# tqch/ddpm-torch

Hardware: AMD Instinct MI355X
Metric: training imgs/s/GPU + 1000-step DDPM samples/s, CIFAR-10 UNet @1/2/4/8 MI355X (higher is better)
Workload: dtype bf16; 1 GPU; configs/cifar10.json UNet (35.7M params), full Trainer.step, B=128 per GPU, 32x32, T=1000, dropout 0.1, Adam+clip+EMA; global_batch=128, rccl_ranks=1, parallelism=dp1

## Files before the change

ddpm-torch_amd/csrc/common.h:

```cpp
#pragma once
#include <hip/hip_runtime.h>
#include <hip/hip_ext.h>
#include <stdint.h>

#define DDPM_OK 0
#define DDPM_ERR_SHAPE 1
#define DDPM_ERR_DTYPE 2
#define DDPM_ERR_ALIGN 3
#define DDPM_ERR_LAUNCH 4
#define DDPM_ERR_NULL 5

#define DDPM_F32 0
#define DDPM_BF16 1

typedef unsigned short bf16_t;

typedef float f32x4 __attribute__((ext_vector_type(4)));
typedef float f32x16 __attribute__((ext_vector_type(16)));
typedef short s16x8 __attribute__((ext_vector_type(8)));
typedef unsigned int u32x4 __attribute__((ext_vector_type(4)));

__device__ __forceinline__ float bf2f(bf16_t v) { return __uint_as_float(((unsigned)v) << 16); }
typedef __attribute__((ext_vector_type(2))) __bf16 hw_bf16x2;
typedef __attribute__((ext_vector_type(2))) float hw_f32x2;
__device__ __forceinline__ unsigned pack_bf2(float lo, float hi) {
    hw_f32x2 v; v.x = lo; v.y = hi;
    return __builtin_bit_cast(unsigned, __builtin_convertvector(v, hw_bf16x2));
}
__device__ __forceinline__ bf16_t f2bf(float f) { return (bf16_t)(pack_bf2(f, 0.f) & 0xffffu); }

template <typename T> struct Elem;
template <> struct Elem<float> {
    static constexpr int VEC = 4;
    __device__ static __forceinline__ float ld(const float* p) { return *p; }
    __device__ static __forceinline__ void st(float* p, float v) { *p = v; }
    __device__ static __forceinline__ void unpack(const u32x4& v, float* f) {
        f[0] = __uint_as_float(v.x); f[1] = __uint_as_float(v.y); f[2] = __uint_as_float(v.z); f[3] = __uint_as_float(v.w);
    }
    __device__ static __forceinline__ u32x4 pack(const float* f) {
        u32x4 v; v.x = __float_as_uint(f[0]); v.y = __float_as_uint(f[1]); v.z = __float_as_uint(f[2]); v.w = __float_as_uint(f[3]);
        return v;
    }
};
template <> struct Elem<bf16_t> {
    static constexpr int VEC = 8;
    __device__ static __forceinline__ float ld(const bf16_t* p) { return bf2f(*p); }
    __device__ static __forceinline__ void st(bf16_t* p, float v) { *p = f2bf(v); }
    __device__ static __forceinline__ void unpack(const u32x4& v, float* f) {
        f[0] = __uint_as_float(v.x << 16); f[1] = __uint_as_float(v.x & 0xffff0000u);
        f[2] = __uint_as_float(v.y << 16); f[3] = __uint_as_float(v.y & 0xffff0000u);
        f[4] = __uint_as_float(v.z << 16); f[5] = __uint_as_float(v.z & 0xffff0000u);
        f[6] = __uint_as_float(v.w << 16); f[7] = __uint_as_float(v.w & 0xffff0000u);
    }
    __device__ static __forceinline__ u32x4 pack(const float* f) {
        u32x4 v; v.x = pack_bf2(f[0], f[1]); v.y = pack_bf2(f[2], f[3]); v.z = pack_bf2(f[4], f[5]); v.w = pack_bf2(f[6], f[7]);
        return v;
    }
};

__device__ __forceinline__ u32x4 ldg16(const void* p) { return *reinterpret_cast<const u32x4*>(p); }
__device__ __forceinline__ void stg16(void* p, const u32x4& v) { *reinterpret_cast<u32x4*>(p) = v; }
__device__ __forceinline__ u32x4 zero16() { u32x4 v; v.x = v.y = v.z = v.w = 0u; return v; }

__device__ __forceinline__ float wave_sum(float v) {
#pragma unroll
    for (int o = 32; o > 0; o >>= 1) v += __shfl_xor(v, o, 64);
    return v;
}
__device__ __forceinline__ float wave_max(float v) {
#pragma unroll
    for (int o = 32; o > 0; o >>= 1) v = fmaxf(v, __shfl_xor(v, o, 64));
    return v;
}

__device__ __forceinline__ float sigmoidf_(float z) { return 1.0f / (1.0f + __expf(-z)); }
__device__ __forceinline__ float siluf_(float z) { return z * sigmoidf_(z); }
__device__ __forceinline__ float silu_fast_(float z) { return z * __builtin_amdgcn_rcpf(1.0f + __expf(-z)); }
__device__ __forceinline__ float silu_gradf_(float z) { float s = sigmoidf_(z); return s * (1.0f + z * (1.0f - s)); }

struct FastDiv {
    unsigned mul, shift, d;
};
__device__ __forceinline__ unsigned fdiv(unsigned n, const FastDiv& f) {
    return (unsigned)(((unsigned long long)n * f.mul) >> f.shift);
}
static inline FastDiv make_fastdiv(unsigned d) {
    FastDiv f; f.d = d ? d : 1; f.mul = 1u << 31; f.shift = 31;
    if (d <= 1) return f;
    unsigned l = 0; while ((1ull << l) < d) ++l;
    f.shift = 31 + l;
    if ((1ull << l) == d) return f;
    f.mul = (unsigned)((1ull << f.shift) / d + 1);
    return f;
}

__device__ __forceinline__ unsigned mix32(unsigned x) {
    x ^= x >> 16; x *= 0x7feb352dU; x ^= x >> 15; x *= 0x846ca68bU; x ^= x >> 16;
    return x;
}
__device__ __forceinline__ unsigned dropout_word(unsigned long long seed, unsigned long long pair) {
    const unsigned lo = (unsigned)pair, hi = (unsigned)(pair >> 32);
    return mix32(lo ^ mix32(hi + (unsigned)seed) ^ (unsigned)(seed >> 32) * 0x9E3779B9u);
}
__device__ __forceinline__ bool dropout_keep(unsigned long long seed, unsigned long long idx, unsigned thresh16) {
    const unsigned w = dropout_word(seed, idx >> 1);
    return ((idx & 1) ? (w >> 16) : (w & 0xffffu)) >= thresh16;
}
__device__ __forceinline__ unsigned dropout_h0(unsigned long long seed) {
    return mix32((unsigned)seed) ^ ((unsigned)(seed >> 32) * 0x9E3779B9u);
}
__device__ __forceinline__ unsigned dropout_word32(unsigned h0, unsigned pair) { return mix32(pair ^ h0); }
static inline unsigned dropout_thresh16(float p) {
    const double th = (double)p * 65536.0;
    return th <= 0 ? 0u : (th >= 65536.0 ? 65536u : (unsigned)(th + 0.5));
}
__device__ __forceinline__ float silu_grad_fast_(float z) {
    const float s = __builtin_amdgcn_rcpf(1.0f + __expf(-z));
    return s * (1.0f + z * (1.0f - s));
}

#include <atomic>
struct DevOnce {
    std::atomic<unsigned long long> mask{0};
    static unsigned long long bit() { int d = 0; (void)hipGetDevice(&d); return 1ull << (d & 63); }
    bool operator!() const { return !(mask.load(std::memory_order_acquire) & bit()); }
    DevOnce& operator=(bool) { mask.fetch_or(bit(), std::memory_order_release); return *this; }
};

struct DdpmLaunchEdge {
    hipStream_t stream = nullptr;
    hipEvent_t event = nullptr;
    bool armed = false;
    bool attached = false;
};
extern thread_local DdpmLaunchEdge g_ddpm_launch_edge;

template <class... P> static inline void ddpm_launch_with_event(DdpmLaunchEdge& edge, void (*kernel)(P...), dim3 grid, dim3 block, unsigned lds,
                                                                hipStream_t st, P... formal) {
    void* args[sizeof...(P) + 1] = {(void*)&formal..., nullptr};
    if (hipExtLaunchKernel((const void*)kernel, grid, block, args, lds, st, nullptr, edge.event, 0) == hipSuccess) edge.attached = true;
}
template <class... P, class... A> static inline void ddpm_launch(void (*kernel)(P...), dim3 grid, dim3 block, unsigned lds, hipStream_t st, A&&... args) {
    static_assert(sizeof...(P) == sizeof...(A), "kernel argument count");
    DdpmLaunchEdge& edge = g_ddpm_launch_edge;
    if (edge.armed && edge.stream == st) ddpm_launch_with_event<P...>(edge, kernel, grid, block, lds, st, static_cast<P>(args)...);
    else kernel<<<grid, block, lds, st>>>(args...);
}
#undef hipLaunchKernelGGL
#define hipLaunchKernelGGL(kernel, grid, block, lds, stream, ...) ddpm_launch(kernel, dim3(grid), dim3(block), (unsigned)(lds), stream, __VA_ARGS__)

static inline int check_launch() { return hipGetLastError() == hipSuccess ? DDPM_OK : DDPM_ERR_LAUNCH; }
static inline bool aligned16(const void* p) { return (((uintptr_t)p) & 15) == 0; }

int ddpm_sumsq_finish_launch(const float* partial, int n, float* total_sq, void* stream);
int ddpm_reserved_cus();
static inline int ddpm_cu_budget(int wanted) { const int left = 256 - ddpm_reserved_cus(); return wanted < left ? wanted : (left > 1 ? left : 1); }
int ddpm_pointwise_launch(const void* x, long long x_ld, const void* w, void* y, long long y_ld, const float* bias, const void* residual,
                          long long res_ld, int accumulate, int M, int N, int K, int dry, void* stream);
int ddpm_edgeconv_few_out_launch(const void* x, long long x_ld, const void* w, void* y, const float* bias, int B, int H, int W, int C, int N,
                                 int dry, void* stream);
int ddpm_edgeconv_few_in_launch(const void* x, long long x_ld, const void* w, void* y, long long y_ld, const float* bias, int B, int H, int W,
                                int C, int N, int dry, void* stream);
int ddpm_conv3x3_stream_launch(const void* x, long long x_ld, const void* w, void* y, long long y_ld, const float* bias, const float* rowbias,
                               long long rowbias_ld, const void* residual, long long res_ld, int accumulate, int B, int H, int W, int C, int N,
                               int upsample, int xcd, int dry, void* stream);
```

ddpm-torch_amd/csrc/elementwise.hip:

```cpp
#include "common.h"
#include <stdlib.h>

static inline int grid_for(long long n, int block = 256, int cap = 256 * 16) {
    long long g = (n + block - 1) / block;
    if (g > cap) g = cap;
    if (g < 1) g = 1;
    return (int)g;
}

__global__ void temb_kernel(const long long* __restrict__ t, const float* __restrict__ freqs, float* __restrict__ out, int B, int dim) {
    const int half = dim / 2;
    for (int i = blockIdx.x * blockDim.x + threadIdx.x; i < B * dim; i += gridDim.x * blockDim.x) {
        const int b = i / dim, j = i - b * dim;
        float v = 0.f;
        if (j < 2 * half) {
            const float arg = __fmul_rn((float)t[b], freqs[j < half ? j : j - half]);
            v = j < half ? sinf(arg) : cosf(arg);
        }
        out[i] = v;
    }
}
extern "C" int ddpm_timestep_embedding(const long long* t, const float* freqs, float* out, int B, int dim, void* stream) {
    if (!t || !out || !freqs) return DDPM_ERR_NULL;
    if (B <= 0 || dim < 4) return DDPM_ERR_SHAPE;
    hipLaunchKernelGGL(temb_kernel, dim3(grid_for((long long)B * dim)), dim3(256), 0, (hipStream_t)stream, t, freqs, out, B, dim);
    return check_launch();
}

template <typename T>
__global__ void nchw_to_nhwc_kernel(const float* __restrict__ x, T* __restrict__ y, int B, int C, int HW, int Cp) {
    const long long n = (long long)B * HW * Cp;
    for (long long i = (long long)blockIdx.x * blockDim.x + threadIdx.x; i < n; i += (long long)gridDim.x * blockDim.x) {
        const int c = (int)(i % Cp);
        const long long bp = i / Cp;
        const int p = (int)(bp % HW);
        const long long b = bp / HW;
        Elem<T>::st(y + i, c < C ? x[(b * C + c) * HW + p] : 0.f);
    }
}
extern "C" int ddpm_nchw_to_nhwc(const float* x, void* y, int B, int C, int HW, int Cp, int dtype, void* stream) {
    if (!x || !y) return DDPM_ERR_NULL;
    if (B <= 0 || C <= 0 || HW <= 0 || Cp < C) return DDPM_ERR_SHAPE;
    const int g = grid_for((long long)B * HW * Cp);
    if (dtype == DDPM_BF16) hipLaunchKernelGGL(nchw_to_nhwc_kernel<bf16_t>, dim3(g), dim3(256), 0, (hipStream_t)stream, x, (bf16_t*)y, B, C, HW, Cp);
    else if (dtype == DDPM_F32) hipLaunchKernelGGL(nchw_to_nhwc_kernel<float>, dim3(g), dim3(256), 0, (hipStream_t)stream, x, (float*)y, B, C, HW, Cp);
    else return DDPM_ERR_DTYPE;
    return check_launch();
}

template <typename T>
__global__ void pack_weight_kernel(const float* __restrict__ w, T* __restrict__ wf, T* __restrict__ wd, int N, int C, int R, int S, int Cp, int Np) {
    const int RS = R * S;
    if (wf) {
        const long long n = (long long)N * RS * Cp;
        for (long long i = (long long)blockIdx.x * blockDim.x + threadIdx.x; i < n; i += (long long)gridDim.x * blockDim.x) {
            const int c = (int)(i % Cp); const long long r1 = i / Cp;
            const int tap = (int)(r1 % RS); const int nn = (int)(r1 / RS);
            Elem<T>::st(wf + i, c < C ? w[((long long)nn * C + c) * RS + tap] : 0.f);
        }
    }
    if (wd) {
        const long long n = (long long)C * RS * Np;
        for (long long i = (long long)blockIdx.x * blockDim.x + threadIdx.x; i < n; i += (long long)gridDim.x * blockDim.x) {
            const int nn = (int)(i % Np); const long long r1 = i / Np;
            const int tap = (int)(r1 % RS); const int c = (int)(r1 / RS);
            Elem<T>::st(wd + i, nn < N ? w[((long long)nn * C + c) * RS + (RS - 1 - tap)] : 0.f);
        }
    }
}
extern "C" int ddpm_pack_weight(const float* w, void* wf, void* wd, int N, int C, int R, int S, int Cp, int Np, int dtype, void* stream) {
    if (!w || (!wf && !wd)) return DDPM_ERR_NULL;
    if (Cp < C || Np < N) return DDPM_ERR_SHAPE;
    const long long big = (long long)(Cp > C ? Cp : C) * R * S * (Np > N ? Np : N);
    const int g = grid_for(big);
    if (dtype == DDPM_BF16) hipLaunchKernelGGL(pack_weight_kernel<bf16_t>, dim3(g), dim3(256), 0, (hipStream_t)stream, w, (bf16_t*)wf, (bf16_t*)wd, N, C, R, S, Cp, Np);
    else if (dtype == DDPM_F32) hipLaunchKernelGGL(pack_weight_kernel<float>, dim3(g), dim3(256), 0, (hipStream_t)stream, w, (float*)wf, (float*)wd, N, C, R, S, Cp, Np);
    else return DDPM_ERR_DTYPE;
    return check_launch();
}

constexpr int PK_T = 32;
template <typename T> __device__ __forceinline__ void pk_store2(T* p, float a, float b);
template <> __device__ __forceinline__ void pk_store2<bf16_t>(bf16_t* p, float a, float b) { *reinterpret_cast<unsigned*>(p) = pack_bf2(a, b); }
template <> __device__ __forceinline__ void pk_store2<float>(float* p, float a, float b) { *reinterpret_cast<float2*>(p) = make_float2(a, b); }

template <typename T, int RS>
__device__ __forceinline__ void pack_tensor(const float* __restrict__ w, T* __restrict__ wf, T* __restrict__ wd, int N, int C, int Cp, int Np, bool up_dgrad,
                                            float* tile) {
    constexpr int pitch = PK_T * RS + 1;
    const int tiles_c = (Cp + PK_T - 1) / PK_T, tiles_n = (Np + PK_T - 1) / PK_T;
    const int tid = threadIdx.x;
    const bool vec_ok = ((long long)C * RS) % 4 == 0 && (((unsigned long long)w) & 15) == 0;
    for (int t = blockIdx.x; t < tiles_c * tiles_n; t += gridDim.x) {
        const int n0 = (t / tiles_c) * PK_T, c0 = (t % tiles_c) * PK_T;
        const int cw = min(PK_T, C - c0);
        __syncthreads();
        constexpr int V = PK_T * RS / 4, KV = PK_T * V / 256;
        static_assert(PK_T * V % 256 == 0, "whole vectors per thread");
        if (cw == PK_T && vec_ok) {
            float4 xv[KV];
#pragma unroll
            for (int k = 0; k < KV; ++k) {
                const int i = tid + 256 * k, nl = i / V, v = i - nl * V;
                xv[k] = n0 + nl < N ? *reinterpret_cast<const float4*>(w + ((long long)(n0 + nl) * C + c0) * RS + 4 * v) : make_float4(0.f, 0.f, 0.f, 0.f);
            }
#pragma unroll
            for (int k = 0; k < KV; ++k) {
                const int i = tid + 256 * k, nl = i / V, v = i - nl * V;
                float* t4 = tile + nl * pitch + 4 * v;
                t4[0] = xv[k].x; t4[1] = xv[k].y; t4[2] = xv[k].z; t4[3] = xv[k].w;
            }
        } else {
            for (int i = tid; i < PK_T * PK_T * RS; i += 256) {
                const int nl = i / (PK_T * RS), rem = i - nl * (PK_T * RS);
                const bool ok = n0 + nl < N && rem < cw * RS;
                tile[nl * pitch + rem] = ok ? w[((long long)(n0 + nl) * C + c0) * RS + rem] : 0.f;
            }
        }
        __syncthreads();
        constexpr bool BF = sizeof(T) == 2;
        if (wf) {
            if constexpr (BF) {
                for (int i = tid; i < PK_T * RS * (PK_T / 8); i += 256) {
                    const int cl = (i % (PK_T / 8)) * 8, r1 = i / (PK_T / 8), tap = r1 % RS, nl = r1 / RS;
                    if (n0 + nl < N && c0 + cl < Cp) {
                        const float* t8 = tile + nl * pitch + cl * RS + tap;
                        u32x4 o;
                        o.x = pack_bf2(t8[0], t8[RS]); o.y = pack_bf2(t8[2 * RS], t8[3 * RS]); o.z = pack_bf2(t8[4 * RS], t8[5 * RS]); o.w = pack_bf2(t8[6 * RS], t8[7 * RS]);
                        *reinterpret_cast<u32x4*>(wf + ((long long)(n0 + nl) * RS + tap) * Cp + c0 + cl) = o;
                    }
                }
            } else {
                for (int i = tid; i < PK_T * RS * (PK_T / 2); i += 256) {
                    const int cl = (i % (PK_T / 2)) * 2, r1 = i / (PK_T / 2), tap = r1 % RS, nl = r1 / RS;
                    if (n0 + nl < N && c0 + cl < Cp)
                        pk_store2<T>(wf + ((long long)(n0 + nl) * RS + tap) * Cp + c0 + cl, tile[nl * pitch + cl * RS + tap], tile[nl * pitch + (cl + 1) * RS + tap]);
                }
            }
        }
        if constexpr (RS == 9) {
            if (wd && up_dgrad) {
                for (int i = tid; i < PK_T * 16 * (PK_T / 2); i += 256) {
                    const int nl = (i % (PK_T / 2)) * 2, r1 = i / (PK_T / 2), tap = r1 % 16, cl = r1 / 16;
                    if (c0 + cl >= C || n0 + nl >= Np) continue;
                    const int P = tap >> 2, Q = tap & 3;
                    float acc0 = 0.f, acc1 = 0.f;
#pragma unroll
                    for (int a = 0; a < 2; ++a)
#pragma unroll
                        for (int b2 = 0; b2 < 2; ++b2) {
                            const int r = P - a, s2 = Q - b2;
                            if (r >= 0 && r < 3 && s2 >= 0 && s2 < 3) {
                                acc0 += tile[nl * pitch + cl * 9 + (8 - (r * 3 + s2))];
                                acc1 += tile[(nl + 1) * pitch + cl * 9 + (8 - (r * 3 + s2))];
                            }
                        }
                    pk_store2<T>(wd + ((long long)(c0 + cl) * 16 + tap) * Np + n0 + nl, acc0, acc1);
                }
                continue;
            }
        }
        if (wd) {
            if constexpr (BF) {
                for (int i = tid; i < PK_T * RS * (PK_T / 8); i += 256) {
                    const int nl = (i % (PK_T / 8)) * 8, r1 = i / (PK_T / 8), tap = r1 % RS, cl = r1 / RS;
                    if (c0 + cl < C && n0 + nl < Np) {
                        const float* t8 = tile + nl * pitch + cl * RS + (RS - 1 - tap);
                        u32x4 o;
                        o.x = pack_bf2(t8[0], t8[pitch]); o.y = pack_bf2(t8[2 * pitch], t8[3 * pitch]); o.z = pack_bf2(t8[4 * pitch], t8[5 * pitch]);
                        o.w = pack_bf2(t8[6 * pitch], t8[7 * pitch]);
                        *reinterpret_cast<u32x4*>(wd + ((long long)(c0 + cl) * RS + tap) * Np + n0 + nl) = o;
                    }
                }
            } else {
                for (int i = tid; i < PK_T * RS * (PK_T / 2); i += 256) {
                    const int nl = (i % (PK_T / 2)) * 2, r1 = i / (PK_T / 2), tap = r1 % RS, cl = r1 / RS;
                    if (c0 + cl < C && n0 + nl < Np)
                        pk_store2<T>(wd + ((long long)(c0 + cl) * RS + tap) * Np + n0 + nl, tile[nl * pitch + cl * RS + (RS - 1 - tap)],
                                     tile[(nl + 1) * pitch + cl * RS + (RS - 1 - tap)]);
                }
            }
        }
    }
}
template <typename T>
__global__ __launch_bounds__(256)
void pack_weight_multi_kernel(const long long* __restrict__ descs) {
    const long long* d = descs + 8 * (long long)blockIdx.y;
    const float* w = reinterpret_cast<const float*>(d[0]);
    T* wf = reinterpret_cast<T*>(d[1]);
    T* wd = reinterpret_cast<T*>(d[2]);
    const int N = (int)d[3], C = (int)d[4], R = (int)d[5] & 0xff, Cp = (int)d[6], Np = (int)d[7];
    const bool up_dgrad = ((int)d[5] & 0x100) != 0;
    __shared__ float tile[PK_T * (PK_T * 9 + 1)];
    if (R == 3) pack_tensor<T, 9>(w, wf, wd, N, C, Cp, Np, up_dgrad, tile);
    else if (R == 1) pack_tensor<T, 1>(w, wf, wd, N, C, Cp, Np, false, tile);
    else if (R == 2) pack_tensor<T, 4>(w, wf, wd, N, C, Cp, Np, false, tile);
}
extern "C" int ddpm_pack_weight_multi(const long long* descs, int n_tensors, int dtype, void* stream) {
    if (!descs) return DDPM_ERR_NULL;
    if (n_tensors <= 0) return DDPM_OK;
    constexpr int pk_blocks = 256;
    if (dtype == DDPM_BF16) hipLaunchKernelGGL(pack_weight_multi_kernel<bf16_t>, dim3(pk_blocks, n_tensors), dim3(256), 0, (hipStream_t)stream, descs);
    else if (dtype == DDPM_F32) hipLaunchKernelGGL(pack_weight_multi_kernel<float>, dim3(pk_blocks, n_tensors), dim3(256), 0, (hipStream_t)stream, descs);
    else return DDPM_ERR_DTYPE;
    return check_launch();
}

__global__ __launch_bounds__(256) void wgrad_unpack_kernel(const float* __restrict__ gpack, float* __restrict__ gflat, const long long* __restrict__ descs, float scale,
                                                            float* __restrict__ sumsq) {
    __shared__ float sh[4];
    const long long* d = descs + 5 * (long long)blockIdx.y;
    const float* src = gpack + d[0];
    float* dst = gflat + d[1];
    const unsigned C = (unsigned)d[3], RS = (unsigned)d[4];
    const unsigned total = (unsigned)(d[2] * C * RS);
    float acc = 0.f;
    if (RS == 1) {
        for (unsigned i = blockIdx.x * blockDim.x + threadIdx.x; i < total; i += gridDim.x * blockDim.x) {
            const float v = src[i] * scale;
            dst[i] = v; acc += v * v;
        }
    } else if (RS == 9 && C % 64 == 0) {
        __shared__ float slab[4][64 * 9];
        const unsigned lane = threadIdx.x & 63, wave = threadIdx.x >> 6, ctiles = C / 64, items = (unsigned)d[2] * ctiles;
        float* mine = slab[wave];
        for (unsigned it = blockIdx.x * 4 + wave; it < items; it += gridDim.x * 4) {
            const unsigned n = it / ctiles, c0 = (it - n * ctiles) * 64;
            float v[9];
#pragma unroll
            for (int tap = 0; tap < 9; ++tap) v[tap] = src[((unsigned long long)n * 9 + tap) * C + c0 + lane] * scale;
#pragma unroll
            for (int tap = 0; tap < 9; ++tap) { mine[lane * 9 + tap] = v[tap]; acc += v[tap] * v[tap]; }
            __builtin_amdgcn_wave_barrier();
            float* out = dst + ((unsigned long long)n * C + c0) * 9;
#pragma unroll
            for (int k = 0; k < 9; ++k) out[k * 64 + lane] = mine[k * 64 + lane];
            __builtin_amdgcn_wave_barrier();
        }
    } else {
        for (unsigned i = blockIdx.x * blockDim.x + threadIdx.x; i < total; i += gridDim.x * blockDim.x) {
            const unsigned nc = i / RS, tap = i - nc * RS;
            const unsigned n = nc / C, c = nc - n * C;
            const float v = src[((unsigned long long)n * RS + tap) * C + c] * scale;
            dst[i] = v; acc += v * v;
        }
    }
    if (sumsq) {
        acc = wave_sum(acc);
        if ((threadIdx.x & 63) == 0) sh[threadIdx.x >> 6] = acc;
        __syncthreads();
        if (threadIdx.x == 0) sumsq[blockIdx.y * gridDim.x + blockIdx.x] = (sh[0] + sh[1]) + (sh[2] + sh[3]);
    }
}
extern "C" int ddpm_wgrad_unpack(const float* gpack, float* gflat, const long long* descs, int n_tensors, float scale, void* stream) {
    if (!gpack || !gflat || !descs) return DDPM_ERR_NULL;
    if (n_tensors <= 0) return DDPM_OK;
    hipLaunchKernelGGL(wgrad_unpack_kernel, dim3(64, n_tensors), dim3(256), 0, (hipStream_t)stream, gpack, gflat, descs, scale, (float*)nullptr);
    return check_launch();
}
extern "C" int ddpm_wgrad_unpack_sumsq(const float* gpack, float* gflat, const long long* descs, int n_tensors, float scale, float* total_sq,
                                       long long total_sq_floats, void* stream) {
    if (!gpack || !gflat || !descs || !total_sq) return DDPM_ERR_NULL;
    if (n_tensors <= 0) return DDPM_OK;
    if (total_sq_floats < 64 + 64ll * n_tensors) return DDPM_ERR_SHAPE;
    hipLaunchKernelGGL(wgrad_unpack_kernel, dim3(64, n_tensors), dim3(256), 0, (hipStream_t)stream, gpack, gflat, descs, scale, total_sq + 64);
    const int rc = check_launch();
    return rc ? rc : ddpm_sumsq_finish_launch(total_sq + 64, 64 * n_tensors, total_sq, stream);
}

__global__ __launch_bounds__(256) void wgrad_reduce_kernel(const long long* __restrict__ table) {
    const long long* d = table + 5 * (long long)blockIdx.y;
    const float* src = reinterpret_cast<const float*>(d[0]);
    float* dst = reinterpret_cast<float*>(d[1]);
    const long long len = d[2], stride = d[4];
    const int copies = (int)d[3];
    const long long nv = len >> 2;
    for (long long v = (long long)blockIdx.x * blockDim.x + threadIdx.x; v < nv; v += (long long)gridDim.x * blockDim.x) {
        const f32x4* col = reinterpret_cast<const f32x4*>(src) + v;
        const long long sv = stride >> 2;
        f32x4 a = col[0];
        int c = 1;
        for (; c + 8 <= copies; c += 8) {
            f32x4 b[8];
#pragma unroll
            for (int k = 0; k < 8; ++k) b[k] = __builtin_nontemporal_load(col + (long long)(c + k) * sv);
#pragma unroll
            for (int k = 0; k < 8; ++k) a += b[k];
        }
        if (c + 4 <= copies) {
            f32x4 b[4];
#pragma unroll
            for (int k = 0; k < 4; ++k) b[k] = __builtin_nontemporal_load(col + (long long)(c + k) * sv);
#pragma unroll
            for (int k = 0; k < 4; ++k) a += b[k];
            c += 4;
        }
        for (; c < copies; ++c) a += __builtin_nontemporal_load(col + (long long)c * sv);
        reinterpret_cast<f32x4*>(dst)[v] = a;
    }
    if (blockIdx.x == 0 && threadIdx.x < (len & 3)) {
        const long long i = (nv << 2) + threadIdx.x;
        float a = src[i];
        for (int c = 1; c < copies; ++c) a += src[(long long)c * stride + i];
        dst[i] = a;
    }
}
extern "C" int ddpm_wgrad_reduce(const long long* table, int n_tensors, void* stream) {
    if (!table) return DDPM_ERR_NULL;
    if (n_tensors <= 0) return DDPM_OK;
    hipLaunchKernelGGL(wgrad_reduce_kernel, dim3(128, n_tensors), dim3(256), 0, (hipStream_t)stream, table);
    return check_launch();
}

__global__ void mt_gather_kernel(const long long* __restrict__ table) {
    const long long* d = table + 4 * (long long)blockIdx.y;
    const float* a = reinterpret_cast<const float*>(d[0]);
    const float* b = reinterpret_cast<const float*>(d[1]);
    float* dst = reinterpret_cast<float*>(d[2]);
    const long long n = d[3];
    if (((d[0] | d[1] | d[2]) & 15) == 0) {
        const long long nv = n >> 2;
        for (long long i = (long long)blockIdx.x * blockDim.x + threadIdx.x; i < nv; i += (long long)gridDim.x * blockDim.x) {
            f32x4 v = reinterpret_cast<const f32x4*>(a)[i];
            if (b) v += reinterpret_cast<const f32x4*>(b)[i];
            reinterpret_cast<f32x4*>(dst)[i] = v;
        }
        for (long long i = (nv << 2) + (long long)blockIdx.x * blockDim.x + threadIdx.x; i < n; i += (long long)gridDim.x * blockDim.x)
            dst[i] = b ? a[i] + b[i] : a[i];
        return;
    }
    for (long long i = (long long)blockIdx.x * blockDim.x + threadIdx.x; i < n; i += (long long)gridDim.x * blockDim.x)
        dst[i] = b ? a[i] + b[i] : a[i];
}
extern "C" int ddpm_mt_gather_f32(const long long* table, int n_tensors, void* stream) {
    if (!table) return DDPM_ERR_NULL;
    if (n_tensors <= 0) return DDPM_OK;
    hipLaunchKernelGGL(mt_gather_kernel, dim3(32, n_tensors), dim3(256), 0, (hipStream_t)stream, table);
    return check_launch();
}

__global__ void q_sample_kernel(const float* __restrict__ x0, const float* __restrict__ noise, const long long* __restrict__ t,
                                const float* __restrict__ ca, const float* __restrict__ cb, float* __restrict__ xt, int B, int n, int T) {
    const long long tot = (long long)B * n;
    for (long long i = (long long)blockIdx.x * blockDim.x + threadIdx.x; i < tot; i += (long long)gridDim.x * blockDim.x) {
        const int b = (int)(i / n);
        const long long tt = t[b];
        xt[i] = (unsigned long long)tt < (unsigned long long)T ? __fadd_rn(__fmul_rn(ca[tt], x0[i]), __fmul_rn(cb[tt], noise[i])) : __builtin_nanf("");
    }
}
extern "C" int ddpm_q_sample(const float* x0, const float* noise, const long long* t, const float* sqrt_ab, const float* sqrt_1mab,
                             float* xt, int B, int n, int T, void* stream) {
    if (!x0 || !noise || !t || !sqrt_ab || !sqrt_1mab || !xt) return DDPM_ERR_NULL;
    if (B <= 0 || n <= 0 || T <= 0) return DDPM_ERR_SHAPE;
    hipLaunchKernelGGL(q_sample_kernel, dim3(grid_for((long long)B * n)), dim3(256), 0, (hipStream_t)stream, x0, noise, t, sqrt_ab, sqrt_1mab, xt, B, n, T);
    return check_launch();
}

__global__ __launch_bounds__(1024) void mse_fwd_kernel(const float* __restrict__ pred, const float* __restrict__ target, float* __restrict__ loss, int n) {
    __shared__ float sh[16];
    const int b = blockIdx.x;
    const float* p = pred + (long long)b * n;
    const float* t = target + (long long)b * n;
    float acc = 0.f;
    const bool al = ((reinterpret_cast<unsigned long long>(p) | reinterpret_cast<unsigned long long>(t)) & 15) == 0;
    const int nv = al ? n >> 2 : 0;
    int i = threadIdx.x;
    for (; i + 3 * (int)blockDim.x < nv; i += 4 * blockDim.x) {
        f32x4 a[4], c[4];
#pragma unroll
        for (int u = 0; u < 4; ++u) { a[u] = reinterpret_cast<const f32x4*>(t)[i + u * blockDim.x]; c[u] = reinterpret_cast<const f32x4*>(p)[i + u * blockDim.x]; }
#pragma unroll
        for (int u = 0; u < 4; ++u) { const f32x4 d = a[u] - c[u]; acc += (d.x * d.x + d.y * d.y) + (d.z * d.z + d.w * d.w); }
    }
    for (; i < nv; i += blockDim.x) { const f32x4 d = reinterpret_cast<const f32x4*>(t)[i] - reinterpret_cast<const f32x4*>(p)[i]; acc += (d.x * d.x + d.y * d.y) + (d.z * d.z + d.w * d.w); }
    for (int j = (nv << 2) + threadIdx.x; j < n; j += blockDim.x) { const float d = t[j] - p[j]; acc += d * d; }
    acc = wave_sum(acc);
    if ((threadIdx.x & 63) == 0) sh[threadIdx.x >> 6] = acc;
    __syncthreads();
    if (threadIdx.x == 0) {
        float tot = 0.f;
        for (int w = 0; w < (int)(blockDim.x >> 6); ++w) tot += sh[w];
        loss[b] = tot / (float)n;
    }
}
__global__ void mse_bwd_kernel(const float* __restrict__ pred, const float* __restrict__ target, const float* __restrict__ gloss,
                               float* __restrict__ gpred, int B, int n) {
    const long long tot = (long long)B * n;
    const float inv = 2.0f / (float)n;
    for (long long i = (long long)blockIdx.x * blockDim.x + threadIdx.x; i < tot; i += (long long)gridDim.x * blockDim.x) {
        const int b = (int)(i / n);
        gpred[i] = (pred[i] - target[i]) * inv * gloss[b];
    }
}
extern "C" int ddpm_mse_fwd(const float* pred, const float* target, float* loss, int B, int n, void* stream) {
    if (!pred || !target || !loss) return DDPM_ERR_NULL;
    if (B <= 0 || n <= 0) return DDPM_ERR_SHAPE;
    hipLaunchKernelGGL(mse_fwd_kernel, dim3(B), dim3(n >= 16384 ? 1024 : 256), 0, (hipStream_t)stream, pred, target, loss, n);
    return check_launch();
}
extern "C" int ddpm_mse_bwd(const float* pred, const float* target, const float* gloss, float* gpred, int B, int n, void* stream) {
    if (!pred || !target || !gloss || !gpred) return DDPM_ERR_NULL;
    if (B <= 0 || n <= 0) return DDPM_ERR_SHAPE;
    hipLaunchKernelGGL(mse_bwd_kernel, dim3(grid_for((long long)B * n)), dim3(256), 0, (hipStream_t)stream, pred, target, gloss, gpred, B, n);
    return check_launch();
}

struct VlbTables { const float *recip, *recip_m1, *coef1, *coef2, *post_logvar, *model_logvar; };
struct VlbCoef { float recip, recip_m1, c1, c2, lv1, lv2; };
__device__ __forceinline__ float vlb_cdf(float z) {
    return 0.5f * (1.0f + tanhf(0.7978845608028654f * (z + 0.044715f * z * z * z)));
}
__device__ __forceinline__ float vlb_cdf_grad(float z) {
    const float th = tanhf(0.7978845608028654f * (z + 0.044715f * z * z * z));
    return 0.5f * (1.0f - th * th) * 0.7978845608028654f * (1.0f + 3.0f * 0.044715f * z * z);
}
__device__ __forceinline__ void vlb_model_mean(const VlbCoef& k, int mean_type, int clip, float xt, float o, float& mean, float& x0p) {
    if (mean_type == 0) x0p = __fsub_rn(__fmul_rn(k.recip, xt), __fmul_rn(k.recip_m1, o));
    else if (mean_type == 1) x0p = o;
    else x0p = __fsub_rn(__fdiv_rn(o, k.c1), __fmul_rn(__fdiv_rn(k.c2, k.c1), xt));
    if (clip) x0p = x0p != x0p ? x0p : fminf(fmaxf(x0p, -1.f), 1.f);
    mean = mean_type == 2 ? o : __fadd_rn(__fmul_rn(k.c1, x0p), __fmul_rn(k.c2, xt));
}
__global__ __launch_bounds__(256) void vlb_terms_kernel(const float* __restrict__ x0, const float* __restrict__ xt, const float* __restrict__ out,
                                                        const long long* __restrict__ t, VlbTables tb, float* __restrict__ loss,
                                                        float* __restrict__ pred_x0, int n, int mean_type, int clip, int T) {
    __shared__ float sh[4];
    const int b = blockIdx.x;
    const long long tt = t[b];
    const long long base = (long long)b * n;
    if ((unsigned long long)tt >= (unsigned long long)T) {
        if (threadIdx.x == 0) loss[b] = __builtin_nanf("");
        if (pred_x0) for (int i = threadIdx.x; i < n; i += blockDim.x) pred_x0[base + i] = __builtin_nanf("");
        return;
    }
    const VlbCoef k{tb.recip[tt], tb.recip_m1[tt], tb.coef1[tt], tb.coef2[tt], tb.post_logvar[tt], tb.model_logvar[tt]};
    const float dlv = k.lv1 - k.lv2, e_dlv = expf(dlv), inv_var2 = expf(-k.lv2), inv_std = expf(-0.5f * k.lv2);
    float acc = 0.f;
    for (int i = threadIdx.x; i < n; i += blockDim.x) {
        const float x = x0[base + i], xti = xt[base + i];
        float mean, x0p;
        vlb_model_mean(k, mean_type, clip, xti, out[base + i], mean, x0p);
        if (pred_x0) pred_x0[base + i] = x0p;
        float term;
        if (tt > 0) {
            const float m1 = __fadd_rn(__fmul_rn(k.c1, x), __fmul_rn(k.c2, xti)), d = m1 - mean;
            term = 0.5f * ((-1.0f - dlv) + d * d * inv_var2 + e_dlv);
        } else {
            const float xc = x - mean;
            const float cu = x > 0.999f ? 1.0f : vlb_cdf(inv_std * (xc + (1.0f / 255.0f)));
            const float cl = x < -0.999f ? 0.0f : vlb_cdf(inv_std * (xc - (1.0f / 255.0f)));
            term = -logf(fmaxf(cu - cl - 1e-12f, 0.f) + 1e-12f);
        }
        acc += term;
    }
    acc = wave_sum(acc);
    if ((threadIdx.x & 63) == 0) sh[threadIdx.x >> 6] = acc;
    __syncthreads();
    if (threadIdx.x == 0) loss[b] = ((sh[0] + sh[1]) + (sh[2] + sh[3])) / (float)n / 0.6931471805599453f;
}
__global__ void vlb_terms_bwd_kernel(const float* __restrict__ x0, const float* __restrict__ xt, const float* __restrict__ out,
                                     const long long* __restrict__ t, VlbTables tb, const float* __restrict__ gloss, float* __restrict__ gout,
                                     int B, int n, int mean_type, int T) {
    const long long tot = (long long)B * n;
    const float inv = 1.0f / ((float)n * 0.6931471805599453f);
    for (long long i = (long long)blockIdx.x * blockDim.x + threadIdx.x; i < tot; i += (long long)gridDim.x * blockDim.x) {
        const int b = (int)(i / n);
        const long long tt = t[b];
        if ((unsigned long long)tt >= (unsigned long long)T) { gout[i] = __builtin_nanf(""); continue; }
        const VlbCoef k{tb.recip[tt], tb.recip_m1[tt], tb.coef1[tt], tb.coef2[tt], tb.post_logvar[tt], tb.model_logvar[tt]};
        const float x = x0[i], xti = xt[i];
        float mean, x0p;
        vlb_model_mean(k, mean_type, 0, xti, out[i], mean, x0p);
        float dterm_dmean;
        if (tt > 0) {
            const float m1 = __fadd_rn(__fmul_rn(k.c1, x), __fmul_rn(k.c2, xti));
            dterm_dmean = -(m1 - mean) * expf(-k.lv2);
        } else {
            const float inv_std = expf(-0.5f * k.lv2), xc = x - mean;
            const float zu = inv_std * (xc + (1.0f / 255.0f)), zl = inv_std * (xc - (1.0f / 255.0f));
            const float cu = x > 0.999f ? 1.0f : vlb_cdf(zu), cl = x < -0.999f ? 0.0f : vlb_cdf(zl);
            const float p = cu - cl - 1e-12f;
            const float dp = -inv_std * ((x > 0.999f ? 0.f : vlb_cdf_grad(zu)) - (x < -0.999f ? 0.f : vlb_cdf_grad(zl)));
            dterm_dmean = p > 0.f ? -dp / (p + 1e-12f) : 0.f;
        }
        const float dmean_dout = mean_type == 0 ? -k.c1 * k.recip_m1 : (mean_type == 1 ? k.c1 : 1.0f);
        gout[i] = gloss[b] * inv * dterm_dmean * dmean_dout;
    }
}
extern "C" int ddpm_vlb_terms(const float* x_0, const float* x_t, const float* model_out, const long long* t,
                              const float* sqrt_recip_ab, const float* sqrt_recip_m1_ab, const float* post_coef1, const float* post_coef2,
                              const float* post_logvar, const float* model_logvar, float* loss, float* pred_x0,
                              int B, int n, int mean_type, int clip, int T, void* stream) {
    if (!x_0 || !x_t || !model_out || !t || !sqrt_recip_ab || !sqrt_recip_m1_ab || !post_coef1 || !post_coef2 || !post_logvar || !model_logvar || !loss)
        return DDPM_ERR_NULL;
    if (B <= 0 || n <= 0 || T <= 0 || mean_type < 0 || mean_type > 2) return DDPM_ERR_SHAPE;
    VlbTables tb{sqrt_recip_ab, sqrt_recip_m1_ab, post_coef1, post_coef2, post_logvar, model_logvar};
    hipLaunchKernelGGL(vlb_terms_kernel, dim3(B), dim3(256), 0, (hipStream_t)stream, x_0, x_t, model_out, t, tb, loss, pred_x0, n, mean_type, clip, T);
    return check_launch();
}
extern "C" int ddpm_vlb_terms_bwd(const float* x_0, const float* x_t, const float* model_out, const long long* t,
                                  const float* sqrt_recip_ab, const float* sqrt_recip_m1_ab, const float* post_coef1, const float* post_coef2,
                                  const float* post_logvar, const float* model_logvar, const float* gloss, float* gout,
                                  int B, int n, int mean_type, int T, void* stream) {
    if (!x_0 || !x_t || !model_out || !t || !sqrt_recip_ab || !sqrt_recip_m1_ab || !post_coef1 || !post_coef2 || !post_logvar || !model_logvar || !gloss || !gout)
        return DDPM_ERR_NULL;
    if (B <= 0 || n <= 0 || T <= 0 || mean_type < 0 || mean_type > 2) return DDPM_ERR_SHAPE;
    VlbTables tb{sqrt_recip_ab, sqrt_recip_m1_ab, post_coef1, post_coef2, post_logvar, model_logvar};
    hipLaunchKernelGGL(vlb_terms_bwd_kernel, dim3(grid_for((long long)B * n)), dim3(256), 0, (hipStream_t)stream, x_0, x_t, model_out, t, tb, gloss, gout,
                       B, n, mean_type, T);
    return check_launch();
}

__global__ void weighted_sum_kernel(const float* __restrict__ x, const float* __restrict__ w, float* __restrict__ out, int n) {
    __shared__ float sh[4];
    float acc = 0.f;
    for (int i = threadIdx.x; i < n; i += blockDim.x) acc += x[i] * w[i];
    acc = wave_sum(acc);
    if ((threadIdx.x & 63) == 0) sh[threadIdx.x >> 6] = acc;
    __syncthreads();
    if (threadIdx.x == 0) out[0] = (sh[0] + sh[1]) + (sh[2] + sh[3]);
}
extern "C" int ddpm_weighted_sum_f32(const float* x, const float* w, float* out, int n, void* stream) {
    if (!x || !w || !out) return DDPM_ERR_NULL;
    if (n <= 0) return DDPM_ERR_SHAPE;
    hipLaunchKernelGGL(weighted_sum_kernel, dim3(1), dim3(256), 0, (hipStream_t)stream, x, w, out, n);
    return check_launch();
}

__global__ __launch_bounds__(256) void atb_f32_kernel(const float* __restrict__ A, long long lda, const float* __restrict__ Bm, long long ldb,
                                                      float* __restrict__ C, long long ldc, int M, int N, int K) {
    __shared__ float sa[32][64 + 4], sb[32][64 + 4];
    const int tid = threadIdx.x, tm = tid >> 4, tn = tid & 15;
    const int m0 = blockIdx.y * 64, n0 = blockIdx.x * 64;
    float acc[4][4];
#pragma unroll
    for (int i = 0; i < 4; ++i)
#pragma unroll
        for (int j = 0; j < 4; ++j) acc[i][j] = 0.f;
    for (int k0 = 0; k0 < K; k0 += 32) {
        for (int e = tid; e < 32 * 64; e += 256) {
            const int kk = e >> 6, c = e & 63, k = k0 + kk;
            sa[kk][c] = (k < K && m0 + c < M) ? A[(long long)k * lda + m0 + c] : 0.f;
            sb[kk][c] = (k < K && n0 + c < N) ? Bm[(long long)k * ldb + n0 + c] : 0.f;
        }
        __syncthreads();
#pragma unroll 8
        for (int kk = 0; kk < 32; ++kk) {
            float a[4], b[4];
#pragma unroll
            for (int i = 0; i < 4; ++i) { a[i] = sa[kk][tm * 4 + i]; b[i] = sb[kk][tn * 4 + i]; }
#pragma unroll
            for (int i = 0; i < 4; ++i)
#pragma unroll
                for (int j = 0; j < 4; ++j) acc[i][j] = fmaf(a[i], b[j], acc[i][j]);
        }
        __syncthreads();
    }
#pragma unroll
    for (int i = 0; i < 4; ++i) {
        const int m = m0 + tm * 4 + i;
        if (m >= M) continue;
#pragma unroll
        for (int j = 0; j < 4; ++j) {
            const int n = n0 + tn * 4 + j;
            if (n < N) C[(long long)m * ldc + n] = acc[i][j];
        }
    }
}
__global__ __launch_bounds__(256) void atb_f32_short_kernel(const float* __restrict__ A, long long lda, const float* __restrict__ Bm, long long ldb,
                                                            float* __restrict__ C, long long ldc, int M, int N, int K) {
    __shared__ __attribute__((aligned(16))) float sa[128][32], sb[128][64];
    const int tid = threadIdx.x, tm = tid >> 4, tn = tid & 15;
    const int m0 = blockIdx.y * 32, n0 = blockIdx.x * 64;
    const f32x4 zero = {0.f, 0.f, 0.f, 0.f};
    f32x4 va[4], vb[8];
#pragma unroll
    for (int i = 0; i < 4; ++i) {
        const int e = tid + 256 * i, kk = e >> 3, c = (e & 7) * 4;
        va[i] = (kk < K && m0 + c < M) ? *reinterpret_cast<const f32x4*>(A + (long long)kk * lda + m0 + c) : zero;
    }
#pragma unroll
    for (int i = 0; i < 8; ++i) {
        const int e = tid + 256 * i, kk = e >> 4, c = (e & 15) * 4;
        vb[i] = (kk < K && n0 + c < N) ? *reinterpret_cast<const f32x4*>(Bm + (long long)kk * ldb + n0 + c) : zero;
    }
#pragma unroll
    for (int i = 0; i < 4; ++i) { const int e = tid + 256 * i; *reinterpret_cast<f32x4*>(&sa[e >> 3][(e & 7) * 4]) = va[i]; }
#pragma unroll
    for (int i = 0; i < 8; ++i) { const int e = tid + 256 * i; *reinterpret_cast<f32x4*>(&sb[e >> 4][(e & 15) * 4]) = vb[i]; }
    __syncthreads();
    float acc[2][4];
#pragma unroll
    for (int i = 0; i < 2; ++i)
#pragma unroll
        for (int j = 0; j < 4; ++j) acc[i][j] = 0.f;
#pragma unroll 8
    for (int kk = 0; kk < K; ++kk) {
        const float a0 = sa[kk][tm * 2], a1 = sa[kk][tm * 2 + 1];
        const f32x4 b = *reinterpret_cast<const f32x4*>(&sb[kk][tn * 4]);
        acc[0][0] = fmaf(a0, b.x, acc[0][0]); acc[0][1] = fmaf(a0, b.y, acc[0][1]); acc[0][2] = fmaf(a0, b.z, acc[0][2]); acc[0][3] = fmaf(a0, b.w, acc[0][3]);
        acc[1][0] = fmaf(a1, b.x, acc[1][0]); acc[1][1] = fmaf(a1, b.y, acc[1][1]); acc[1][2] = fmaf(a1, b.z, acc[1][2]); acc[1][3] = fmaf(a1, b.w, acc[1][3]);
    }
#pragma unroll
    for (int i = 0; i < 2; ++i) {
        const int m = m0 + tm * 2 + i, n = n0 + tn * 4;
        if (m < M && n < N) *reinterpret_cast<f32x4*>(C + (long long)m * ldc + n) = f32x4{acc[i][0], acc[i][1], acc[i][2], acc[i][3]};
    }
}
extern "C" int ddpm_atb_f32(const float* a, long long lda, const float* b, long long ldb, float* c, long long ldc, int M, int N, int K, void* stream) {
    if (!a || !b || !c) return DDPM_ERR_NULL;
    if (M <= 0 || N <= 0 || K <= 0 || lda < M || ldb < N || ldc < N) return DDPM_ERR_SHAPE;
    const bool vec = ((M | N | (int)(lda & 3) | (int)(ldb & 3) | (int)(ldc & 3)) & 3) == 0 && aligned16(a) && aligned16(b) && aligned16(c);
    if (K <= 128 && vec)
        hipLaunchKernelGGL(atb_f32_short_kernel, dim3((N + 63) / 64, (M + 31) / 32), dim3(256), 0, (hipStream_t)stream, a, lda, b, ldb, c, ldc, M, N, K);
    else
        hipLaunchKernelGGL(atb_f32_kernel, dim3((N + 63) / 64, (M + 63) / 64), dim3(256), 0, (hipStream_t)stream, a, lda, b, ldb, c, ldc, M, N, K);
    return check_launch();
}

struct StepTables { const float *recip, *recip_m1, *coef1, *coef2, *logvar; };
__global__ void p_step_kernel(const float* __restrict__ x_t, const float* __restrict__ out, const float* __restrict__ z,
                              const long long* __restrict__ t, StepTables tb, float* __restrict__ x_prev, float* __restrict__ pred_x0,
                              int B, int n, int mean_type, int clip, int T) {
    const long long tot = (long long)B * n;
    for (long long i = (long long)blockIdx.x * blockDim.x + threadIdx.x; i < tot; i += (long long)gridDim.x * blockDim.x) {
        const int b = (int)(i / n);
        const long long tt = t[b];
        if ((unsigned long long)tt >= (unsigned long long)T) {
            x_prev[i] = __builtin_nanf("");
            if (pred_x0) pred_x0[i] = __builtin_nanf("");
            continue;
        }
        const float xt = x_t[i], o = out[i];
        float x0, mean;
        if (mean_type == 0) {
            x0 = __fsub_rn(__fmul_rn(tb.recip[tt], xt), __fmul_rn(tb.recip_m1[tt], o));
        } else if (mean_type == 1) {
            x0 = o;
        } else {
            const float c1 = tb.coef1[tt], c2 = tb.coef2[tt];
            x0 = __fsub_rn(__fdiv_rn(o, c1), __fmul_rn(__fdiv_rn(c2, c1), xt));
        }
        if (clip) x0 = x0 != x0 ? x0 : fminf(fmaxf(x0, -1.f), 1.f);
        if (mean_type == 2) mean = o;
        else mean = __fadd_rn(__fmul_rn(tb.coef1[tt], x0), __fmul_rn(tb.coef2[tt], xt));
        const float mask = tt > 0 ? 1.f : 0.f;
        const float sd = expf(__fmul_rn(0.5f, tb.logvar[tt]));
        x_prev[i] = __fadd_rn(mean, __fmul_rn(__fmul_rn(mask, sd), z[i]));
        if (pred_x0) pred_x0[i] = x0;
    }
}
extern "C" int ddpm_p_sample_step(const float* x_t, const float* model_out, const float* z, const long long* t,
                                  const float* sqrt_recip_ab, const float* sqrt_recip_m1_ab, const float* post_coef1, const float* post_coef2,
                                  const float* logvar, float* x_prev, float* pred_x0, int B, int n, int mean_type, int clip, int T, void* stream) {
    if (!x_t || !model_out || !z || !t || !x_prev || !sqrt_recip_ab || !sqrt_recip_m1_ab || !post_coef1 || !post_coef2 || !logvar) return DDPM_ERR_NULL;
    if (B <= 0 || n <= 0 || T <= 0 || mean_type < 0 || mean_type > 2) return DDPM_ERR_SHAPE;
    StepTables tb{sqrt_recip_ab, sqrt_recip_m1_ab, post_coef1, post_coef2, logvar};
    hipLaunchKernelGGL(p_step_kernel, dim3(grid_for((long long)B * n)), dim3(256), 0, (hipStream_t)stream, x_t, model_out, z, t, tb, x_prev, pred_x0, B, n, mean_type, clip, T);
    return check_launch();
}

__global__ void gather_i64_kernel(const long long* __restrict__ idx, const long long* __restrict__ map, long long* __restrict__ out, int B) {
    const int i = blockIdx.x * blockDim.x + threadIdx.x;
    if (i < B) out[i] = map[idx[i]];
}
__global__ void add_i64_kernel(long long* __restrict__ t, int B, long long delta) {
    const int i = blockIdx.x * blockDim.x + threadIdx.x;
    if (i < B) t[i] += delta;
}
__global__ __launch_bounds__(256) void gather_rows_kernel(const float* __restrict__ table, const long long* __restrict__ idx, float* __restrict__ out,
                                                          int row_len, int table_rows) {
    const long long t = idx[blockIdx.x];
    const bool ok = t >= 0 && t < table_rows;
    const f32x4* src = reinterpret_cast<const f32x4*>(table + (ok ? t : 0) * row_len);
    f32x4* dst = reinterpret_cast<f32x4*>(out + (long long)blockIdx.x * row_len);
    const f32x4 poison = (f32x4)(__builtin_nanf(""));
    for (int i = threadIdx.x; i < row_len / 4; i += 256) dst[i] = ok ? src[i] : poison;
}
extern "C" int ddpm_gather_rows_f32(const float* table, const long long* idx, float* out, int rows, int row_len, int table_rows, void* stream) {
    if (!table || !idx || !out) return DDPM_ERR_NULL;
    if (rows <= 0 || row_len <= 0 || row_len % 4 || table_rows <= 0) return DDPM_ERR_SHAPE;
    if (!aligned16(table) || !aligned16(out)) return DDPM_ERR_ALIGN;
    hipLaunchKernelGGL(gather_rows_kernel, dim3(rows), dim3(256), 0, (hipStream_t)stream, table, idx, out, row_len, table_rows);
    return check_launch();
}
extern "C" int ddpm_gather_i64(const long long* idx, const long long* map, long long* out, int B, void* stream) {
    if (!idx || !map || !out) return DDPM_ERR_NULL;
    hipLaunchKernelGGL(gather_i64_kernel, dim3((B + 255) / 256), dim3(256), 0, (hipStream_t)stream, idx, map, out, B);
    return check_launch();
}
extern "C" int ddpm_add_i64(long long* t, int B, long long delta, void* stream) {
    if (!t) return DDPM_ERR_NULL;
    hipLaunchKernelGGL(add_i64_kernel, dim3((B + 255) / 256), dim3(256), 0, (hipStream_t)stream, t, B, delta);
    return check_launch();
}

__global__ void silu_fwd_kernel(const float* __restrict__ x, float* __restrict__ y, long long n) {
    for (long long i = (long long)blockIdx.x * blockDim.x + threadIdx.x; i < n; i += (long long)gridDim.x * blockDim.x) y[i] = siluf_(x[i]);
}
__global__ void silu_bwd_kernel(const float* __restrict__ x, const float* __restrict__ dy, float* __restrict__ dx, long long n, int accumulate) {
    for (long long i = (long long)blockIdx.x * blockDim.x + threadIdx.x; i < n; i += (long long)gridDim.x * blockDim.x) {
        const float g = dy[i] * silu_gradf_(x[i]);
        dx[i] = accumulate ? dx[i] + g : g;
    }
}
extern "C" int ddpm_silu_fwd(const float* x, float* y, long long n, void* stream) {
    if (!x || !y) return DDPM_ERR_NULL;
    hipLaunchKernelGGL(silu_fwd_kernel, dim3(grid_for(n)), dim3(256), 0, (hipStream_t)stream, x, y, n);
    return check_launch();
}
extern "C" int ddpm_silu_bwd(const float* x, const float* dy, float* dx, long long n, int accumulate, void* stream) {
    if (!x || !dy || !dx) return DDPM_ERR_NULL;
    hipLaunchKernelGGL(silu_bwd_kernel, dim3(grid_for(n)), dim3(256), 0, (hipStream_t)stream, x, dy, dx, n, accumulate);
    return check_launch();
}

template <typename T>
__global__ void colsum_kernel(const T* __restrict__ dy, long long ld, float* __restrict__ per_sample, long long ps_ld,
                              float* __restrict__ total, int HW, int C, int pix_per_slab) {
    constexpr int VEC = Elem<T>::VEC;
    __shared__ float sh[8192];
    const int b = blockIdx.y;
    const int cx = threadIdx.x, py = threadIdx.y;
    const int t = threadIdx.y * blockDim.x + threadIdx.x, nt = blockDim.x * blockDim.y;
    const int p0 = blockIdx.x * pix_per_slab, p1 = min(HW, p0 + pix_per_slab);
    const int c_base = blockIdx.z * blockDim.x * VEC;
    dy += c_base;
    if (per_sample) per_sample += c_base;
    if (total) total += c_base;
    C = min(C - c_base, (int)blockDim.x * VEC);
    const bool live = cx * VEC < C;
    float acc[VEC];
#pragma unroll
    for (int j = 0; j < VEC; ++j) acc[j] = 0.f;
    const T* base = dy + (long long)b * HW * ld + cx * VEC;
    if (live) {
#pragma unroll 4
        for (int p = p0 + py; p < p1; p += blockDim.y) {
            float f[VEC];
            Elem<T>::unpack(ldg16(base + (long long)p * ld), f);
#pragma unroll
            for (int j = 0; j < VEC; ++j) acc[j] += f[j];
        }
#pragma unroll
        for (int j = 0; j < VEC; ++j) sh[py * C + cx * VEC + j] = acc[j];
    }
    __syncthreads();
    for (int c = t; c < C; c += nt) {
        float a = 0.f;
        for (int r = 0; r < (int)blockDim.y; ++r) a += sh[r * C + c];
        if (per_sample) atomicAdd(per_sample + (long long)b * ps_ld + c, a);
        if (total) atomicAdd(total + c, a);
    }
}
extern "C" int ddpm_colsum(const void* dy, long long ld, float* per_sample, long long ps_ld, float* total, int B, int HW, int C, int dtype, void* stream) {
    if (!dy || (!per_sample && !total)) return DDPM_ERR_NULL;
    const int vec = dtype == DDPM_BF16 ? 8 : 4;
    if (C % vec || ld % vec || C / vec > 256 * 64) return DDPM_ERR_SHAPE;
    if (!aligned16(dy)) return DDPM_ERR_ALIGN;
    const int Z = (C / vec + 255) / 256;
    const int cv = Z > 1 ? 256 : C / vec;
    int py = 1024 / cv; if (py > HW) py = HW; if (py < 1) py = 1;
    int S = (256 + B - 1) / B;
    const int maxS = (HW + 4 * py - 1) / (4 * py);
    if (S > maxS) S = maxS;
    if (S < 1) S = 1;
    const int pps = (HW + S - 1) / S;
    S = (HW + pps - 1) / pps;
    if (dtype == DDPM_BF16) hipLaunchKernelGGL(colsum_kernel<bf16_t>, dim3(S, B, Z), dim3(cv, py), 0, (hipStream_t)stream, (const bf16_t*)dy, ld, per_sample, ps_ld, total, HW, C, pps);
    else if (dtype == DDPM_F32) hipLaunchKernelGGL(colsum_kernel<float>, dim3(S, B, Z), dim3(cv, py), 0, (hipStream_t)stream, (const float*)dy, ld, per_sample, ps_ld, total, HW, C, pps);
    else return DDPM_ERR_DTYPE;
    return check_launch();
}

template <typename T>
__global__ void resample2x_kernel(const T* __restrict__ x, long long x_ld, T* __restrict__ y, long long y_ld, int B, int H, int W, int C, int up,
                                  float scale, int accumulate) {
    constexpr int VEC = Elem<T>::VEC;
    const int cv = C / VEC;
    const long long n = (long long)B * H * W * cv;
    for (long long i = (long long)blockIdx.x * blockDim.x + threadIdx.x; i < n; i += (long long)gridDim.x * blockDim.x) {
        const int c = (int)(i % cv) * VEC;
        long long r = i / cv;
        const int w = (int)(r % W); r /= W;
        const int h = (int)(r % H); const long long b = r / H;
        const long long small = (b * H + h) * W + w, big = ((b * 2 * H + 2 * h) * 2 * W) + 2 * w;
        if (!up) {
            float acc[VEC];
#pragma unroll
            for (int j = 0; j < VEC; ++j) acc[j] = 0.f;
#pragma unroll
            for (int a = 0; a < 2; ++a)
#pragma unroll
                for (int bb = 0; bb < 2; ++bb) {
                    float f[VEC];
                    Elem<T>::unpack(ldg16(x + (big + (long long)a * 2 * W + bb) * x_ld + c), f);
#pragma unroll
                    for (int j = 0; j < VEC; ++j) acc[j] += f[j];
                }
#pragma unroll
            for (int j = 0; j < VEC; ++j) acc[j] *= scale;
            T* o = y + small * y_ld + c;
            if (accumulate) {
                float f[VEC];
                Elem<T>::unpack(ldg16(o), f);
#pragma unroll
                for (int j = 0; j < VEC; ++j) acc[j] += f[j];
            }
            stg16(o, Elem<T>::pack(acc));
        } else {
            float v[VEC];
            Elem<T>::unpack(ldg16(x + small * x_ld + c), v);
#pragma unroll
            for (int j = 0; j < VEC; ++j) v[j] *= scale;
#pragma unroll
            for (int a = 0; a < 2; ++a)
#pragma unroll
                for (int bb = 0; bb < 2; ++bb) {
                    T* o = y + (big + (long long)a * 2 * W + bb) * y_ld + c;
                    float out[VEC];
#pragma unroll
                    for (int j = 0; j < VEC; ++j) out[j] = v[j];
                    if (accumulate) {
                        float f[VEC];
                        Elem<T>::unpack(ldg16(o), f);
#pragma unroll
                        for (int j = 0; j < VEC; ++j) out[j] += f[j];
                    }
                    stg16(o, Elem<T>::pack(out));
                }
        }
    }
}
extern "C" int ddpm_resample2x_nhwc(const void* x, long long x_ld, void* y, long long y_ld, int B, int H, int W, int C, int up, float scale,
                                    int accumulate, int dtype, void* stream) {
    if (!x || !y) return DDPM_ERR_NULL;
    if (B <= 0 || H <= 0 || W <= 0 || C <= 0 || (up != 0 && up != 1)) return DDPM_ERR_SHAPE;
    const int vec = dtype == DDPM_BF16 ? 8 : 4;
    if (dtype != DDPM_BF16 && dtype != DDPM_F32) return DDPM_ERR_DTYPE;
    if (C % vec || x_ld % vec || y_ld % vec || x_ld < C || y_ld < C) return DDPM_ERR_SHAPE;
    if (!aligned16(x) || !aligned16(y)) return DDPM_ERR_ALIGN;
    const int g = grid_for((long long)B * H * W * (C / vec));
    if (dtype == DDPM_BF16)
        hipLaunchKernelGGL(resample2x_kernel<bf16_t>, dim3(g), dim3(256), 0, (hipStream_t)stream, (const bf16_t*)x, x_ld, (bf16_t*)y, y_ld, B, H, W, C, up, scale, accumulate);
    else
        hipLaunchKernelGGL(resample2x_kernel<float>, dim3(g), dim3(256), 0, (hipStream_t)stream, (const float*)x, x_ld, (float*)y, y_ld, B, H, W, C, up, scale, accumulate);
    return check_launch();
}

template <typename T>
__global__ void upsample_bwd_kernel(const T* __restrict__ dyu, T* __restrict__ dx, int B, int H, int W, int C, long long dx_ld, int accumulate) {
    constexpr int VEC = Elem<T>::VEC;
    const int cv = C / VEC;
    const long long n = (long long)B * H * W * cv;
    for (long long i = (long long)blockIdx.x * blockDim.x + threadIdx.x; i < n; i += (long long)gridDim.x * blockDim.x) {
        const int c = (int)(i % cv) * VEC;
        long long r = i / cv;
        const int x = (int)(r % W); r /= W;
        const int y = (int)(r % H); const long long b = r / H;
        float acc[VEC];
#pragma unroll
        for (int j = 0; j < VEC; ++j) acc[j] = 0.f;
#pragma unroll
        for (int dy = 0; dy < 2; ++dy)
#pragma unroll
            for (int dxx = 0; dxx < 2; ++dxx) {
                float f[VEC];
                Elem<T>::unpack(ldg16(dyu + (((b * 2 * H + 2 * y + dy) * 2 * W) + 2 * x + dxx) * C + c), f);
#pragma unroll
                for (int j = 0; j < VEC; ++j) acc[j] += f[j];
            }
        T* o = dx + ((b * H + y) * W + x) * dx_ld + c;
        if (accumulate) {
            float f[VEC];
            Elem<T>::unpack(ldg16(o), f);
#pragma unroll
            for (int j = 0; j < VEC; ++j) acc[j] += f[j];
        }
        stg16(o, Elem<T>::pack(acc));
    }
}
extern "C" int ddpm_upsample2x_bwd(const void* dy_up, void* dx, long long dx_ld, int B, int H, int W, int C, int accumulate, int dtype, void* stream) {
    if (!dy_up || !dx) return DDPM_ERR_NULL;
    const int vec = dtype == DDPM_BF16 ? 8 : 4;
    if (C % vec || dx_ld % vec) return DDPM_ERR_SHAPE;
    const int g = grid_for((long long)B * H * W * (C / vec));
    if (dtype == DDPM_BF16) hipLaunchKernelGGL(upsample_bwd_kernel<bf16_t>, dim3(g), dim3(256), 0, (hipStream_t)stream, (const bf16_t*)dy_up, (bf16_t*)dx, B, H, W, C, dx_ld, accumulate);
    else if (dtype == DDPM_F32) hipLaunchKernelGGL(upsample_bwd_kernel<float>, dim3(g), dim3(256), 0, (hipStream_t)stream, (const float*)dy_up, (float*)dx, B, H, W, C, dx_ld, accumulate);
    else return DDPM_ERR_DTYPE;
    return check_launch();
}

template <typename T>
__global__ void add_kernel(const T* __restrict__ x, long long x_ld, T* __restrict__ y, long long y_ld, long long rows, int C, int accumulate) {
    constexpr int VEC = Elem<T>::VEC;
    const int cv = C / VEC;
    const long long n = rows * cv;
    for (long long i = (long long)blockIdx.x * blockDim.x + threadIdx.x; i < n; i += (long long)gridDim.x * blockDim.x) {
        const int c = (int)(i % cv) * VEC; const long long r = i / cv;
        float a[VEC];
        Elem<T>::unpack(ldg16(x + r * x_ld + c), a);
        if (accumulate) {
            float b[VEC];
            Elem<T>::unpack(ldg16(y + r * y_ld + c), b);
#pragma unroll
            for (int j = 0; j < VEC; ++j) a[j] += b[j];
        }
        stg16(y + r * y_ld + c, Elem<T>::pack(a));
    }
}
extern "C" int ddpm_add_rows(const void* x, long long x_ld, void* y, long long y_ld, long long rows, int C, int accumulate, int dtype, void* stream) {
    if (!x || !y) return DDPM_ERR_NULL;
    const int vec = dtype == DDPM_BF16 ? 8 : 4;
    if (C % vec || x_ld % vec || y_ld % vec) return DDPM_ERR_SHAPE;
    const int g = grid_for(rows * (C / vec));
    if (dtype == DDPM_BF16) hipLaunchKernelGGL(add_kernel<bf16_t>, dim3(g), dim3(256), 0, (hipStream_t)stream, (const bf16_t*)x, x_ld, (bf16_t*)y, y_ld, rows, C, accumulate);
    else if (dtype == DDPM_F32) hipLaunchKernelGGL(add_kernel<float>, dim3(g), dim3(256), 0, (hipStream_t)stream, (const float*)x, x_ld, (float*)y, y_ld, rows, C, accumulate);
    else return DDPM_ERR_DTYPE;
    return check_launch();
}

template <typename T>
__global__ void softmax_fwd_kernel(const float* __restrict__ s, T* __restrict__ p, long long rows, int L) {
    const int lane = threadIdx.x & 63;
    const long long row = (long long)blockIdx.x * (blockDim.x >> 6) + (threadIdx.x >> 6);
    if (row >= rows) return;
    const float* sr = s + row * L;
    float m = -INFINITY;
    for (int i = lane; i < L; i += 64) m = fmaxf(m, sr[i]);
    m = wave_max(m);
    float sum = 0.f;
    for (int i = lane; i < L; i += 64) sum += __expf(sr[i] - m);
    sum = wave_sum(sum);
    const float inv = 1.0f / sum;
    for (int i = lane; i < L; i += 64) Elem<T>::st(p + row * L + i, __expf(sr[i] - m) * inv);
}
template <typename T>
__global__ void softmax_bwd_kernel(const T* __restrict__ p, const float* __restrict__ dp, T* __restrict__ ds, long long rows, int L) {
    const int lane = threadIdx.x & 63;
    const long long row = (long long)blockIdx.x * (blockDim.x >> 6) + (threadIdx.x >> 6);
    if (row >= rows) return;
    float dot = 0.f;
    for (int i = lane; i < L; i += 64) dot += Elem<T>::ld(p + row * L + i) * dp[row * L + i];
    dot = wave_sum(dot);
    for (int i = lane; i < L; i += 64) {
        const float pv = Elem<T>::ld(p + row * L + i);
        Elem<T>::st(ds + row * L + i, pv * (dp[row * L + i] - dot));
    }
}
extern "C" int ddpm_softmax_fwd(const float* s, void* p, long long rows, int L, int dtype, void* stream) {
    if (!s || !p) return DDPM_ERR_NULL;
    const int g = (int)((rows + 3) / 4);
    if (dtype == DDPM_BF16) hipLaunchKernelGGL(softmax_fwd_kernel<bf16_t>, dim3(g), dim3(256), 0, (hipStream_t)stream, s, (bf16_t*)p, rows, L);
    else if (dtype == DDPM_F32) hipLaunchKernelGGL(softmax_fwd_kernel<float>, dim3(g), dim3(256), 0, (hipStream_t)stream, s, (float*)p, rows, L);
    else return DDPM_ERR_DTYPE;
    return check_launch();
}
extern "C" int ddpm_softmax_bwd(const void* p, const float* dp, void* ds, long long rows, int L, int dtype, void* stream) {
    if (!p || !dp || !ds) return DDPM_ERR_NULL;
    const int g = (int)((rows + 3) / 4);
    if (dtype == DDPM_BF16) hipLaunchKernelGGL(softmax_bwd_kernel<bf16_t>, dim3(g), dim3(256), 0, (hipStream_t)stream, (const bf16_t*)p, dp, (bf16_t*)ds, rows, L);
    else if (dtype == DDPM_F32) hipLaunchKernelGGL(softmax_bwd_kernel<float>, dim3(g), dim3(256), 0, (hipStream_t)stream, (const float*)p, dp, (float*)ds, rows, L);
    else return DDPM_ERR_DTYPE;
    return check_launch();
}

__global__ void dropout_mask_kernel(float* __restrict__ mask, long long n, unsigned long long seed, unsigned thresh16) {
    for (long long i = (long long)blockIdx.x * blockDim.x + threadIdx.x; i < n; i += (long long)gridDim.x * blockDim.x)
        mask[i] = dropout_keep(seed, (unsigned long long)i, thresh16) ? 1.f : 0.f;
}
extern "C" int ddpm_dropout_mask(float* mask, long long n, float p, unsigned long long seed, void* stream) {
    if (!mask) return DDPM_ERR_NULL;
    hipLaunchKernelGGL(dropout_mask_kernel, dim3(grid_for(n)), dim3(256), 0, (hipStream_t)stream, mask, n, seed, dropout_thresh16(p));
    return check_launch();
}
```

ddpm-torch_amd/csrc/optim.hip:

```cpp
#include "common.h"

__global__ void sumsq_kernel(const float* __restrict__ g, long long n, float* __restrict__ partial) {
    __shared__ float sh[4];
    float acc = 0.f;
    for (long long i = (long long)blockIdx.x * blockDim.x + threadIdx.x; i < n; i += (long long)gridDim.x * blockDim.x) acc += g[i] * g[i];
    acc = wave_sum(acc);
    if ((threadIdx.x & 63) == 0) sh[threadIdx.x >> 6] = acc;
    __syncthreads();
    if (threadIdx.x == 0) partial[blockIdx.x] = sh[0] + sh[1] + sh[2] + sh[3];
}
__global__ void sum_partials_kernel(const float* __restrict__ partial, int nblk, float* __restrict__ out) {
    __shared__ float sh[4];
    float acc = 0.f;
    for (int i = threadIdx.x; i < nblk; i += blockDim.x) acc += partial[i];
    acc = wave_sum(acc);
    if ((threadIdx.x & 63) == 0) sh[threadIdx.x >> 6] = acc;
    __syncthreads();
    if (threadIdx.x == 0) out[0] += sh[0] + sh[1] + sh[2] + sh[3];
}
extern "C" int ddpm_sumsq_accumulate(const float* g, long long n, float* total_sq, float* workspace, void* stream) {
    if (!g || !total_sq || !workspace) return DDPM_ERR_NULL;
    if (n <= 0) return DDPM_OK;
    long long want = (n + 255) / 256;
    const int nblk = (int)(want > 1024 ? 1024 : want);
    hipLaunchKernelGGL(sumsq_kernel, dim3(nblk), dim3(256), 0, (hipStream_t)stream, g, n, workspace);
    hipLaunchKernelGGL(sum_partials_kernel, dim3(1), dim3(256), 0, (hipStream_t)stream, workspace, nblk, total_sq);
    return check_launch();
}

__global__ void adam_ema_kernel(float* __restrict__ p, const float* __restrict__ g, float* __restrict__ m, float* __restrict__ v,
                                float* __restrict__ shadow, long long n, const float* __restrict__ total_sq, float max_norm,
                                float lr, float beta1, float beta2, float eps, float bc1, float bc2, float ema_w) {
    float clip = 1.f;
    if (total_sq && max_norm > 0.f) {
        const float c = max_norm / (sqrtf(total_sq[0]) + 1e-6f);
        clip = c < 1.f ? c : 1.f;
    }
    const float step = lr / bc1;
    const float sqrt_bc2 = sqrtf(bc2);
    for (long long i = (long long)blockIdx.x * blockDim.x + threadIdx.x; i < n; i += (long long)gridDim.x * blockDim.x) {
        const float gi = g[i] * clip;
        const float mi = beta1 * m[i] + (1.f - beta1) * gi;
        const float vi = beta2 * v[i] + (1.f - beta2) * gi * gi;
        m[i] = mi; v[i] = vi;
        const float denom = sqrtf(vi) / sqrt_bc2 + eps;
        const float pi = p[i] - step * (mi / denom);
        p[i] = pi;
        if (shadow) shadow[i] += ema_w * (pi - shadow[i]);
    }
}
extern "C" int ddpm_adam_ema_step(float* p, const float* g, float* m, float* v, float* shadow, long long n, const float* total_sq,
                                  float max_norm, float lr, float beta1, float beta2, float eps, float bias_corr1, float bias_corr2,
                                  float ema_w, void* stream) {
    if (!p || !g || !m || !v) return DDPM_ERR_NULL;
    if (n <= 0) return DDPM_OK;
    long long want = (n + 255) / 256;
    const int nblk = (int)(want > 4096 ? 4096 : want);
    hipLaunchKernelGGL(adam_ema_kernel, dim3(nblk), dim3(256), 0, (hipStream_t)stream, p, g, m, v, shadow, n, total_sq, max_norm, lr, beta1, beta2,
                       eps, bias_corr1, bias_corr2, ema_w);
    return check_launch();
}

constexpr int MT_SUMSQ_LANES = 64;
__global__ __launch_bounds__(1024) void sumsq_finish_kernel(const float* __restrict__ partial, int n, float* __restrict__ total_sq) {
    __shared__ float sh[1024];
    float acc = 0.f;
    for (int i = threadIdx.x; i < n; i += 1024) acc += partial[i];
    sh[threadIdx.x] = acc;
    __syncthreads();
    for (int w = 512; w > 0; w >>= 1) {
        if ((int)threadIdx.x < w) sh[threadIdx.x] += sh[threadIdx.x + w];
        __syncthreads();
    }
    if (threadIdx.x < MT_SUMSQ_LANES) total_sq[threadIdx.x] = threadIdx.x == 0 ? sh[0] : 0.f;
}
int ddpm_sumsq_finish_launch(const float* partial, int n, float* total_sq, void* stream) {
    hipLaunchKernelGGL(sumsq_finish_kernel, dim3(1), dim3(1024), 0, (hipStream_t)stream, partial, n, total_sq);
    return check_launch();
}
constexpr int MT_SUMSQ_BLOCKS = 16;
__global__ void mt_sumsq_kernel(const long long* __restrict__ table, float* __restrict__ partial) {
    __shared__ float sh[4];
    const long long* row = table + 6 * (long long)blockIdx.y;
    const float* g = reinterpret_cast<const float*>(row[1]);
    const long long n = row[5];
    float acc = 0.f;
    const long long nv = (reinterpret_cast<unsigned long long>(g) & 15) == 0 ? n >> 2 : 0;
    for (long long i = (long long)blockIdx.x * blockDim.x + threadIdx.x; i < nv; i += (long long)gridDim.x * blockDim.x) {
        const float4 v = reinterpret_cast<const float4*>(g)[i];
        acc += (v.x * v.x + v.y * v.y) + (v.z * v.z + v.w * v.w);
    }
    for (long long i = (nv << 2) + (long long)blockIdx.x * blockDim.x + threadIdx.x; i < n; i += (long long)gridDim.x * blockDim.x) acc += g[i] * g[i];
    acc = wave_sum(acc);
    if ((threadIdx.x & 63) == 0) sh[threadIdx.x >> 6] = acc;
    __syncthreads();
    if (threadIdx.x == 0) partial[blockIdx.y * gridDim.x + blockIdx.x] = (sh[0] + sh[1]) + (sh[2] + sh[3]);
}
__global__ void mt_adam_ema_kernel(const long long* __restrict__ table, const float* __restrict__ total_sq, float max_norm, float lr,
                                   float beta1, float beta2, float eps, float bc1, float bc2, float ema_w, const float* __restrict__ hyper) {
    if (hyper) { lr = hyper[0]; bc1 = hyper[1]; bc2 = hyper[2]; ema_w = hyper[3]; }
    const long long* row = table + 6 * (long long)blockIdx.y;
    float* p = reinterpret_cast<float*>(row[0]);
    const float* g = reinterpret_cast<const float*>(row[1]);
    float* m = reinterpret_cast<float*>(row[2]);
    float* v = reinterpret_cast<float*>(row[3]);
    float* shadow = reinterpret_cast<float*>(row[4]);
    const long long n = row[5];
    float clip = 1.f;
    if (total_sq && max_norm > 0.f) {
        float tot = 0.f;
        for (int i = 0; i < MT_SUMSQ_LANES; ++i) tot += total_sq[i];
        const float c = max_norm / (sqrtf(tot) + 1e-6f);
        clip = c < 1.f ? c : 1.f;
    }
    const float step = lr / bc1;
    const float sqrt_bc2 = sqrtf(bc2);
    auto upd = [&](float& pi, float gi, float& mi, float& vi, float& si) {
        gi *= clip;
        mi = beta1 * mi + (1.f - beta1) * gi;
        vi = beta2 * vi + (1.f - beta2) * gi * gi;
        const float denom = sqrtf(vi) / sqrt_bc2 + eps;
        pi = pi - step * (mi / denom);
        si += ema_w * (pi - si);
    };
    const unsigned long long al = reinterpret_cast<unsigned long long>(p) | reinterpret_cast<unsigned long long>(g) | reinterpret_cast<unsigned long long>(m) |
                                  reinterpret_cast<unsigned long long>(v) | reinterpret_cast<unsigned long long>(shadow);
    const long long nv = (al & 15) == 0 ? n >> 2 : 0;
    for (long long i = (long long)blockIdx.x * blockDim.x + threadIdx.x; i < nv; i += (long long)gridDim.x * blockDim.x) {
        float4 p4 = reinterpret_cast<float4*>(p)[i], m4 = reinterpret_cast<float4*>(m)[i], v4 = reinterpret_cast<float4*>(v)[i];
        const float4 g4 = reinterpret_cast<const float4*>(g)[i];
        float4 s4 = shadow ? reinterpret_cast<float4*>(shadow)[i] : make_float4(0.f, 0.f, 0.f, 0.f);
        upd(p4.x, g4.x, m4.x, v4.x, s4.x); upd(p4.y, g4.y, m4.y, v4.y, s4.y);
        upd(p4.z, g4.z, m4.z, v4.z, s4.z); upd(p4.w, g4.w, m4.w, v4.w, s4.w);
        reinterpret_cast<float4*>(p)[i] = p4; reinterpret_cast<float4*>(m)[i] = m4; reinterpret_cast<float4*>(v)[i] = v4;
        if (shadow) reinterpret_cast<float4*>(shadow)[i] = s4;
    }
    for (long long i = (nv << 2) + (long long)blockIdx.x * blockDim.x + threadIdx.x; i < n; i += (long long)gridDim.x * blockDim.x) {
        float pi = p[i], mi = m[i], vi = v[i], si = shadow ? shadow[i] : 0.f;
        upd(pi, g[i], mi, vi, si);
        p[i] = pi; m[i] = mi; v[i] = vi;
        if (shadow) shadow[i] = si;
    }
}
extern "C" int ddpm_mt_sumsq_slots(int n_tensors) { return MT_SUMSQ_LANES + 64 * (n_tensors > 0 ? n_tensors : 0); }
extern "C" int ddpm_mt_grad_sumsq(const long long* table, int n_tensors, float* total_sq, long long total_sq_floats, void* stream) {
    if (!table || !total_sq) return DDPM_ERR_NULL;
    if (n_tensors <= 0) return DDPM_OK;
    if (total_sq_floats < ddpm_mt_sumsq_slots(n_tensors)) return DDPM_ERR_SHAPE;
    hipLaunchKernelGGL(mt_sumsq_kernel, dim3(MT_SUMSQ_BLOCKS, n_tensors), dim3(256), 0, (hipStream_t)stream, table, total_sq + MT_SUMSQ_LANES);
    const int rc = check_launch();
    return rc ? rc : ddpm_sumsq_finish_launch(total_sq + MT_SUMSQ_LANES, MT_SUMSQ_BLOCKS * n_tensors, total_sq, stream);
}
extern "C" int ddpm_mt_adam_ema(const long long* table, int n_tensors, const float* total_sq, float max_norm, float lr, float beta1,
                                float beta2, float eps, float bias_corr1, float bias_corr2, float ema_w, const float* hyper_dev, void* stream) {
    if (!table) return DDPM_ERR_NULL;
    if (n_tensors <= 0) return DDPM_OK;
    hipLaunchKernelGGL(mt_adam_ema_kernel, dim3(32, n_tensors), dim3(256), 0, (hipStream_t)stream, table, total_sq, max_norm, lr, beta1, beta2, eps,
                       bias_corr1, bias_corr2, ema_w, hyper_dev);
    return check_launch();
}
```

ddpm-torch_amd/csrc/plan.hip:

```cpp
#include "common.h"
#include "../../include/ddpm_hip.h"
#include "../../include/ddpm_hip_debug.h"

#include <cstring>
#include <mutex>
#include <type_traits>
#include <utility>
#include <vector>

namespace {

typedef unsigned long long word_t;

template <class T> inline T from_word(word_t w) {
    if constexpr (std::is_pointer<T>::value) {
        return reinterpret_cast<T>(static_cast<uintptr_t>(w));
    } else if constexpr (std::is_same<T, float>::value) {
        const unsigned u = static_cast<unsigned>(w);
        float f;
        std::memcpy(&f, &u, 4);
        return f;
    } else {
        return static_cast<T>(w);
    }
}

typedef int (*thunk_t)(const word_t*);

template <class... A, size_t... I> inline int invoke(int (*fn)(A...), const word_t* w, std::index_sequence<I...>) {
    return fn(from_word<A>(w[I])...);
}
template <class... A> constexpr int arity(int (*)(A...)) { return (int)sizeof...(A); }
template <class... A> inline int invoke_all(int (*fn)(A...), const word_t* w) { return invoke(fn, w, std::index_sequence_for<A...>{}); }

enum EntryKind { EP_KERNELS, EP_ENQUEUES, EP_EDGE };

struct EntryPoint {
    const char* name;
    thunk_t thunk;
    int nargs;
    EntryKind kind;
};

#define EP(fn) {#fn, [](const word_t* w) -> int { return invoke_all(&fn, w); }, arity(&fn), EP_KERNELS}
#define EP_AS(fn, kind) {#fn, [](const word_t* w) -> int { return invoke_all(&fn, w); }, arity(&fn), kind}

}

extern "C" int ddpm_stream_order(void* waiter, void* signaller);
extern "C" int ddpm_fill_zero(void* p, long long bytes, void* stream);

namespace {

const EntryPoint kEntryPoints[] = {
    EP(ddpm_conv2d_nhwc), EP(ddpm_conv2d_wgrad_nhwc), EP(ddpm_conv3x3_wgrad_nhwc), EP(ddpm_conv3x3_wgrad_up_nhwc), EP(ddpm_conv1x1_wgrad_nhwc),
    EP(ddpm_wgrad_reduce), EP(ddpm_wgrad_unpack), EP(ddpm_wgrad_unpack_sumsq), EP(ddpm_gemm),
    EP(ddpm_attention_fwd), EP(ddpm_attention_fwd_lse), EP(ddpm_attention_bwd), EP(ddpm_groupnorm_silu_fwd),
    EP(ddpm_groupnorm_silu_bwd), EP(ddpm_timestep_embedding), EP(ddpm_nchw_to_nhwc), EP(ddpm_pack_weight), EP(ddpm_pack_weight_multi),
    EP(ddpm_q_sample), EP(ddpm_mse_fwd), EP(ddpm_mse_bwd), EP(ddpm_weighted_sum_f32), EP(ddpm_atb_f32), EP(ddpm_p_sample_step), EP(ddpm_vlb_terms), EP(ddpm_vlb_terms_bwd), EP(ddpm_gather_i64),
    EP(ddpm_add_i64), EP(ddpm_gather_rows_f32), EP(ddpm_silu_fwd), EP(ddpm_silu_bwd), EP(ddpm_colsum), EP(ddpm_upsample2x_bwd), EP(ddpm_resample2x_nhwc),
    EP(ddpm_add_rows), EP(ddpm_softmax_fwd), EP(ddpm_softmax_bwd), EP(ddpm_sumsq_accumulate), EP(ddpm_adam_ema_step), EP(ddpm_mt_grad_sumsq),
    EP(ddpm_mt_adam_ema), EP(ddpm_mt_gather_f32), EP(ddpm_mfma_probe), EP(ddpm_copy_probe), EP(ddpm_dropout_mask), EP_AS(ddpm_stream_order, EP_EDGE), EP_AS(ddpm_fill_zero, EP_ENQUEUES),
    EP(ddpm_toy_time_table), EP(ddpm_toy_decoder_fwd), EP(ddpm_toy_decoder_bwd), EP(ddpm_toy_time_table_bwd),
    EP(ddpm_manifold_kth_f16), EP(ddpm_manifold_cover_f16),
};
constexpr int kNumEntryPoints = (int)(sizeof(kEntryPoints) / sizeof(kEntryPoints[0]));

enum Mode : unsigned char { RUN, PRODUCER, WAIT, RECORD, SKIP };

struct Entry {
    thunk_t thunk;
    int first_word;
    int ep;
    Mode mode = RUN;
    int producer = -1;
};

struct Plan {
    std::vector<Entry> entries;
    std::vector<word_t> words;
    std::vector<int> segment_end;
    std::vector<hipEvent_t> bound;
    size_t resolved_entries = 0, resolved_cuts = 0;
    int failed_index = -1;
    int failed_status = 0;
};

constexpr int kRing = 2048;
struct EventRing {
    hipEvent_t ev[kRing];
    std::atomic<unsigned> next{0};
    bool ready = false;
};
EventRing g_rings[64];
std::mutex g_ring_mutex;

EventRing* ring_of_device() {
    int dev = 0;
    if (hipGetDevice(&dev) != hipSuccess) return nullptr;
    EventRing& r = g_rings[dev & 63];
    std::lock_guard<std::mutex> lock(g_ring_mutex);
    if (!r.ready) {
        for (int i = 0; i < kRing; ++i)
            if (hipEventCreateWithFlags(&r.ev[i], hipEventDisableTiming) != hipSuccess) return nullptr;
        r.ready = true;
    }
    return &r;
}
inline hipEvent_t next_event(EventRing& r) { return r.ev[r.next.fetch_add(1, std::memory_order_relaxed) % kRing]; }

inline int record_and_wait(EventRing& r, hipStream_t waiter, hipStream_t signaller) {
    const hipEvent_t e = next_event(r);
    if (hipEventRecord(e, signaller) != hipSuccess) return DDPM_ERR_LAUNCH;
    if (hipStreamWaitEvent(waiter, e, 0) != hipSuccess) return DDPM_ERR_LAUNCH;
    return DDPM_OK;
}

void resolve(Plan* p) {
    const int n = (int)p->entries.size();
    const word_t* words = p->words.data();
    for (Entry& e : p->entries) { e.mode = RUN; e.producer = -1; }
    size_t seg = 0;
    int first = 0;
    for (int i = 0; i < n; ++i) {
        while (seg < p->segment_end.size() && p->segment_end[seg] <= i) first = p->segment_end[seg++];
        Entry& e = p->entries[i];
        if (kEntryPoints[e.ep].kind != EP_EDGE) continue;
        const word_t waiter = words[e.first_word], signaller = words[e.first_word + 1];
        if (waiter == signaller) continue;
        e.mode = RECORD;
        for (int j = i - 1; j >= first; --j) {
            const Entry& q = p->entries[j];
            const EntryPoint& ep = kEntryPoints[q.ep];
            if (ep.kind == EP_EDGE) {
                if (words[q.first_word] == waiter && words[q.first_word + 1] == signaller) { e.mode = SKIP; break; }
                if (words[q.first_word] == signaller && words[q.first_word + 1] != signaller) break;
                continue;
            }
            if (words[q.first_word + ep.nargs - 1] != signaller) continue;
            if (ep.kind == EP_KERNELS) { e.mode = WAIT; e.producer = j; }
            break;
        }
        if (e.mode == WAIT) p->entries[e.producer].mode = PRODUCER;
    }
    p->bound.assign(n, nullptr);
    p->resolved_entries = p->entries.size();
    p->resolved_cuts = p->segment_end.size();
}

}

thread_local DdpmLaunchEdge g_ddpm_launch_edge;

extern "C" {

int ddpm_stream_order(void* waiter, void* signaller) {
    if (waiter == signaller) return DDPM_OK;
    EventRing* r = ring_of_device();
    if (!r) return DDPM_ERR_LAUNCH;
    return record_and_wait(*r, (hipStream_t)waiter, (hipStream_t)signaller);
}

int ddpm_fill_zero(void* p, long long bytes, void* stream) {
    if (bytes < 0) return DDPM_ERR_SHAPE;
    if (bytes == 0) return DDPM_OK;
    if (!p) return DDPM_ERR_NULL;
    return hipMemsetAsync(p, 0, (size_t)bytes, (hipStream_t)stream) == hipSuccess ? DDPM_OK : DDPM_ERR_LAUNCH;
}

void* ddpm_plan_create(void) { return new Plan(); }

int ddpm_plan_destroy(void* plan) {
    delete static_cast<Plan*>(plan);
    return DDPM_OK;
}

int ddpm_plan_append(void* plan, const char* entry, const unsigned long long* words, int n_words) {
    if (!plan || !entry || (!words && n_words > 0)) return -DDPM_ERR_NULL;
    Plan* p = static_cast<Plan*>(plan);
    for (int i = 0; i < kNumEntryPoints; ++i) {
        if (std::strcmp(kEntryPoints[i].name, entry) != 0) continue;
        if (kEntryPoints[i].nargs != n_words) return -DDPM_ERR_SHAPE;
        Entry e;
        e.thunk = kEntryPoints[i].thunk;
        e.first_word = (int)p->words.size();
        e.ep = i;
        p->words.insert(p->words.end(), words, words + n_words);
        p->entries.push_back(e);
        return (int)p->entries.size() - 1;
    }
    return -DDPM_ERR_SHAPE;
}

int ddpm_plan_cut(void* plan) {
    if (!plan) return -DDPM_ERR_NULL;
    Plan* p = static_cast<Plan*>(plan);
    p->segment_end.push_back((int)p->entries.size());
    return (int)p->segment_end.size() - 1;
}

int ddpm_plan_segments(void* plan) {
    if (!plan) return -DDPM_ERR_NULL;
    Plan* p = static_cast<Plan*>(plan);
    const int closed = (int)p->segment_end.size();
    const int last_end = closed ? p->segment_end.back() : 0;
    return closed + ((int)p->entries.size() > last_end ? 1 : 0);
}

int ddpm_plan_entries(void* plan) { return plan ? (int)static_cast<Plan*>(plan)->entries.size() : -DDPM_ERR_NULL; }

int ddpm_plan_run(void* plan, int segment) {
    if (!plan) return DDPM_ERR_NULL;
    Plan* p = static_cast<Plan*>(plan);
    const int closed = (int)p->segment_end.size();
    if (segment < 0 || segment > closed) return DDPM_ERR_SHAPE;
    const int first = segment ? p->segment_end[segment - 1] : 0;
    const int last = segment < closed ? p->segment_end[segment] : (int)p->entries.size();
    if (p->resolved_entries != p->entries.size() || p->resolved_cuts != p->segment_end.size()) resolve(p);
    const word_t* words = p->words.data();
    const Entry* e = p->entries.data();
    EventRing* ring = nullptr;
    DdpmLaunchEdge& arm = g_ddpm_launch_edge;
    for (int i = first; i < last; ++i) {
        const word_t* w = words + e[i].first_word;
        int rc = DDPM_OK;
        if (e[i].mode == RUN) {
            rc = e[i].thunk(w);
        } else if (e[i].mode == SKIP) {
            continue;
        } else {
            if (!ring && !(ring = ring_of_device())) rc = DDPM_ERR_LAUNCH;
            else if (e[i].mode == PRODUCER) {
                arm.stream = (hipStream_t)(uintptr_t)w[kEntryPoints[e[i].ep].nargs - 1];
                arm.event = next_event(*ring);
                arm.attached = false;
                arm.armed = true;
                rc = e[i].thunk(w);
                arm.armed = false;
                p->bound[i] = arm.attached ? arm.event : nullptr;
            } else {
                const hipStream_t waiter = (hipStream_t)(uintptr_t)w[0], signaller = (hipStream_t)(uintptr_t)w[1];
                const hipEvent_t ev = e[i].mode == WAIT ? p->bound[e[i].producer] : nullptr;
                if (ev) rc = hipStreamWaitEvent(waiter, ev, 0) == hipSuccess ? DDPM_OK : DDPM_ERR_LAUNCH;
                else rc = record_and_wait(*ring, waiter, signaller);
            }
        }
        if (rc != DDPM_OK) {
            p->failed_index = i;
            p->failed_status = rc;
            return rc;
        }
    }
    return DDPM_OK;
}

const char* ddpm_plan_failed_entry(void* plan, int* index) {
    if (!plan) return nullptr;
    Plan* p = static_cast<Plan*>(plan);
    if (index) *index = p->failed_index;
    return p->failed_index < 0 ? nullptr : kEntryPoints[p->entries[p->failed_index].ep].name;
}

int ddpm_plan_entry_arity(const char* entry) {
    if (!entry) return -1;
    for (int i = 0; i < kNumEntryPoints; ++i)
        if (std::strcmp(kEntryPoints[i].name, entry) == 0) return kEntryPoints[i].nargs;
    return -1;
}

}
```

ddpm-torch_amd/ddpm_torch/_hip.py:

```python
import ctypes
import os
from ctypes import c_float, c_int, c_longlong, c_ulonglong, c_void_p

import torch

_HERE = os.path.dirname(os.path.abspath(__file__))
LIB_PATH = os.environ.get("DDPM_HIP_LIB") or os.path.join(os.path.dirname(_HERE), "csrc", "libddpm_hip.so")

F32, BF16 = 0, 1
_ERR = {1: "bad shape / divisibility", 2: "unsupported dtype", 3: "misaligned pointer or pitch",
        4: "kernel launch failed", 5: "null pointer"}

P, I, L, F, U = c_void_p, c_int, c_longlong, c_float, c_ulonglong

PROTOTYPES = {
    "ddpm_conv2d_nhwc": [P, L, P, P, L, P, P, L, P, L] + [I] * 14 + [I, I, I, P, P, I, P],
    "ddpm_conv2d_wgrad_nhwc": [P, L, P, L, P, L] + [I] * 17 + [P],
    "ddpm_wgrad_effective_splits": [I, I, I],
    "ddpm_conv3x3_wgrad_splits": [I, I, I, I, I, I],
    "ddpm_conv3x3_wgrad_nhwc": [P, L, P, L, P, L, P, L, I, I, I, I, I, I, I, I, P],
    "ddpm_conv3x3_wgrad_up_nhwc": [P, L, P, L, P, L, P, L, I, I, I, I, I, I, I, I, P],
    "ddpm_conv1x1_wgrad_splits": [I, I, I],
    "ddpm_conv1x1_wgrad_nhwc": [P, L, P, L, P, L, P, L, I, I, I, I, I, P],
    "ddpm_wgrad_reduce": [P, I, P],
    "ddpm_wgrad_unpack": [P, P, P, I, F, P],
    "ddpm_wgrad_unpack_sumsq": [P, P, P, I, F, P, L, P],
    "ddpm_gemm": [P, L, L, I, P, L, L, I, P, L, L, P, P, L, L, I, I, I, I, F, I, I, I, I, P],
    "ddpm_groupnorm_silu_fwd": [P, L, P, L, P, P, P, P, I, I, I, I, F, I, F, U, P, I, P],
    "ddpm_groupnorm_silu_bwd": [P, L, P, L, P, L, P, P, P, P, P, P, I, I, I, I, I, F, U, P, I, P, L, P, L, I, P],
    "ddpm_gn_workspace_floats": [I, I, I, I, I],
    "ddpm_conv2d_variant": [L, L] + [I] * 18,
    "ddpm_conv2d_wgrad_variant": [L, L] + [I] * 17,
    "ddpm_gemm_variant": [L, I, L, I, L, I, I, I, I, I, I, I],
    "ddpm_attention_fwd": [P, L, P, L, I, I, I, F, I, P],
    "ddpm_attention_fwd_lse": [P, L, P, L, P, I, I, I, F, I, P],
    "ddpm_attention_bwd": [P, L, P, L, P, L, P, P, P, L, I, I, I, F, I, P],
    "ddpm_timestep_embedding": [P, P, P, I, I, P],
    "ddpm_nchw_to_nhwc": [P, P, I, I, I, I, I, P],
    "ddpm_pack_weight": [P, P, P, I, I, I, I, I, I, I, P],
    "ddpm_pack_weight_multi": [P, I, I, P],
    "ddpm_q_sample": [P, P, P, P, P, P, I, I, I, P],
    "ddpm_mse_fwd": [P, P, P, I, I, P],
    "ddpm_mse_bwd": [P, P, P, P, I, I, P],
    "ddpm_weighted_sum_f32": [P, P, P, I, P],
    "ddpm_atb_f32": [P, L, P, L, P, L, I, I, I, P],
    "ddpm_p_sample_step": [P, P, P, P, P, P, P, P, P, P, P, I, I, I, I, I, P],
    "ddpm_vlb_terms": [P] * 12 + [I, I, I, I, I, P],
    "ddpm_vlb_terms_bwd": [P] * 12 + [I, I, I, I, P],
    "ddpm_gather_i64": [P, P, P, I, P],
    "ddpm_add_i64": [P, I, L, P],
    "ddpm_gather_rows_f32": [P, P, P, I, I, I, P],
    "ddpm_silu_fwd": [P, P, L, P],
    "ddpm_silu_bwd": [P, P, P, L, I, P],
    "ddpm_colsum": [P, L, P, L, P, I, I, I, I, P],
    "ddpm_upsample2x_bwd": [P, P, L, I, I, I, I, I, I, P],
    "ddpm_resample2x_nhwc": [P, L, P, L, I, I, I, I, I, F, I, I, P],
    "ddpm_add_rows": [P, L, P, L, L, I, I, I, P],
    "ddpm_softmax_fwd": [P, P, L, I, I, P],
    "ddpm_softmax_bwd": [P, P, P, L, I, I, P],
    "ddpm_dropout_mask": [P, L, F, U, P],
    "ddpm_mfma_probe": [P, I, I, P],
    "ddpm_mt_sumsq_slots": [I],
    "ddpm_conv3x3_wgrad_variant": [I, I, I, I, I],
    "ddpm_wgrad3x3_ws_last_fault": [P],
    "ddpm_mt_grad_sumsq": [P, I, P, L, P],
    "ddpm_mt_adam_ema": [P, I, P, F, F, F, F, F, F, F, F, P, P],
    "ddpm_mt_gather_f32": [P, I, P],
    "ddpm_sumsq_accumulate": [P, L, P, P, P],
    "ddpm_adam_ema_step": [P, P, P, P, P, L, P, F, F, F, F, F, F, F, F, P],
    "ddpm_conv3x3_pc_last_fault": [P],
    "ddpm_set_reserved_cus": [I],
    "ddpm_get_reserved_cus": [],
    "ddpm_copy_probe": [P, P, L, I, P],
    "ddpm_toy_time_table": [P, P, P, P, P, P, I, I, P],
    "ddpm_toy_decoder_fwd": [P] * 16 + [I] * 5 + [P],
    "ddpm_toy_decoder_bwd": [P] * 19 + [L] + [I] * 5 + [P],
    "ddpm_toy_time_table_bwd": [P] * 7 + [L, I, I, I, P],
    "ddpm_manifold_kth_f16": [P, L, I, P, L, I, I, I, P, P, L, P],
    "ddpm_manifold_cover_f16": [P, L, I, P, L, I, I, P, P, P, L, P],
    "ddpm_stream_order": [P, P],
    "ddpm_fill_zero": [P, L, P],
    "ddpm_plan_create": [],
    "ddpm_plan_destroy": [P],
    "ddpm_plan_append": [P, ctypes.c_char_p, P, I],
    "ddpm_plan_cut": [P],
    "ddpm_plan_segments": [P],
    "ddpm_plan_entries": [P],
    "ddpm_plan_run": [P, I],
    "ddpm_plan_failed_entry": [P, P],
    "ddpm_plan_entry_arity": [ctypes.c_char_p],
}
RESTYPES = {"ddpm_gn_workspace_floats": c_longlong, "ddpm_plan_create": c_void_p, "ddpm_plan_failed_entry": ctypes.c_char_p}

_lib = None


def lib():
    global _lib
    if _lib is None:
        if not os.path.exists(LIB_PATH):
            raise RuntimeError(
                f"ddpm_torch (MI355X build): HIP library not found at {LIB_PATH}. "
                "Build it with `python ddpm-torch_amd/csrc/build.py` — there is no CPU fallback.")
        handle = ctypes.CDLL(LIB_PATH)
        for name, argtypes in PROTOTYPES.items():
            try:
                fn = getattr(handle, name)
            except AttributeError as e:
                raise RuntimeError(f"{LIB_PATH} does not export {name}; rebuild it") from e
            fn.argtypes = argtypes
            fn.restype = RESTYPES.get(name, c_int)
        _lib = handle
    return _lib


SUMSQ_MAX_TENSORS = 8192
SUMSQ_FLOATS = 64 + 64 * SUMSQ_MAX_TENSORS


def _invoke(name, args):
    rc = getattr(lib(), name)(*args)
    if rc != 0:
        raise RuntimeError(f"{name} failed: {_ERR.get(rc, rc)}")


_recorder = None


def call(name, *args):
    if _recorder is not None:
        _recorder.add(name, args)
    _invoke(name, args)


def record_into(plan):
    global _recorder
    prev, _recorder = _recorder, plan
    return prev


def retain(t):
    if _recorder is not None and _recorder.retains:
        _recorder.keep.append(t)
    return t


_raw_stream = getattr(torch._C, "_cuda_getCurrentRawStream", None)


_routed = None


def route_stream(handle):
    global _routed
    prev, _routed = _routed, handle
    return prev


def stream():
    if _routed is not None:
        return _routed
    if _raw_stream is not None:
        return _raw_stream(torch.cuda.current_device())
    return torch.cuda.current_stream().cuda_stream


def dt(t):
    if t.dtype == torch.float32:
        return F32
    if t.dtype == torch.bfloat16:
        return BF16
    raise TypeError(f"unsupported dtype {t.dtype}")


def require_cuda(*tensors):
    for t in tensors:
        if t is not None and not t.is_cuda:
            raise RuntimeError("ddpm_torch (MI355X build) runs on CUDA/HIP tensors only; "
                               "got a CPU tensor and there is no CPU fallback")


def on_device(t):
    return t.is_cuda


def ptr(t):
    return 0 if t is None else t.data_ptr()
```

ddpm-torch_amd/ddpm_torch/_plan.py:

```python
import contextlib
import ctypes
import gc
import struct

import torch

from . import _hip

__all__ = ["LaunchPlan"]

_MASK64 = (1 << 64) - 1


def _words(name, args):
    types = _hip.PROTOTYPES[name]
    if len(types) != len(args):
        raise TypeError(f"{name}: {len(args)} arguments recorded, {len(types)} declared")
    out = []
    for ty, v in zip(types, args):
        if ty is _hip.F:
            out.append(struct.unpack("<I", struct.pack("<f", float(v)))[0])
        elif ty is _hip.I:
            out.append(int(v) & 0xFFFFFFFF)
        else:
            out.append((0 if v is None else int(v)) & _MASK64)
    return out


class LaunchPlan:
    def __init__(self, device):
        self.device = torch.device(device)
        self.segments = [[]]
        self.callbacks = []
        self.keep = []
        self.retains = self.device.type != "cuda"
        self.pool = None
        self._c = None
        self.recorded = False
        self.build_error = None

    def add(self, name, args):
        self.segments[-1].append((name, args))

    def cut(self, fn):
        self.callbacks.append(fn)
        self.segments.append([])
        fn()

    def record(self, body):
        assert not self.recorded
        on_gpu = self.device.type == "cuda"
        if on_gpu:
            self.pool = torch.cuda.MemPool()
            scope = torch.cuda.use_mem_pool(self.pool, device=self.device)
        else:
            scope = contextlib.nullcontext()
        gc.collect()
        gc_was_on = gc.isenabled()
        gc.disable()
        prev = _hip.record_into(self)
        try:
            with scope:
                body(self.cut)
        finally:
            _hip.record_into(prev)
            if gc_was_on:
                gc.enable()
        if on_gpu:
            try:
                count = getattr(self.pool, "use_count", None)
                if callable(count) and count() < 1:
                    raise RuntimeError("the plan's MemPool lost its last reference when the recording scope closed")
                self._build_native()
            except Exception as e:
                self.build_error = f"{type(e).__name__}: {e}"
        self.recorded = True
        return self

    def _build_native(self):
        lib = _hip.lib()
        h = lib.ddpm_plan_create()
        if not h:
            raise RuntimeError("ddpm_plan_create failed")
        self._c = ctypes.c_void_p(h)
        for i, seg in enumerate(self.segments):
            for name, args in seg:
                w = _words(name, args)
                arr = (ctypes.c_ulonglong * len(w))(*w)
                rc = lib.ddpm_plan_append(self._c, name.encode(), ctypes.cast(arr, ctypes.c_void_p), len(w))
                if rc < 0:
                    raise RuntimeError(f"ddpm_plan_append({name}) failed: the executor does not know this entry point with {len(w)} arguments")
            if i + 1 < len(self.segments):
                lib.ddpm_plan_cut(self._c)

    def replay(self):
        if self._c is not None:
            lib = _hip.lib()
            for i in range(len(self.segments)):
                rc = lib.ddpm_plan_run(self._c, i)
                if rc != 0:
                    idx = ctypes.c_int(-1)
                    name = lib.ddpm_plan_failed_entry(self._c, ctypes.cast(ctypes.pointer(idx), ctypes.c_void_p))
                    raise RuntimeError(f"launch plan: {name.decode() if name else '?'} (entry {idx.value}) failed: {_hip._ERR.get(rc, rc)}")
                if i < len(self.callbacks):
                    self.callbacks[i]()
        else:
            for i, seg in enumerate(self.segments):
                for name, args in seg:
                    _hip._invoke(name, args)
                if i < len(self.callbacks):
                    self.callbacks[i]()

    @property
    def launches(self):
        return sum(len(s) for s in self.segments)

    def __del__(self):
        c, self._c = getattr(self, "_c", None), None
        if c is not None:
            try:
                _hip.lib().ddpm_plan_destroy(c)
            except Exception:
                pass
```

include/ddpm_hip.h:

```cpp
#ifndef DDPM_HIP_H
#define DDPM_HIP_H
#ifdef __cplusplus
extern "C" {
#endif

int ddpm_conv2d_nhwc(const void* x, long long x_ld, const void* w, void* y, long long y_ld,
                     const float* bias, const float* rowbias, long long rowbias_ld,
                     const void* residual, long long res_ld,
                     int B, int H, int W, int C, int Ho, int Wo, int N, int R, int S,
                     int stride, int pad_t, int pad_l, int upsample, int dilate,
                     int accumulate, int out_mode, int splits, float* splitk_ws, unsigned* splitk_cnt,
                     int dtype, void* stream);

int ddpm_conv2d_wgrad_nhwc(const void* dy, long long dy_ld, const void* x, long long x_ld, float* dw, long long slab_stride,
                           int B, int H, int W, int C, int Creal, int Ho, int Wo, int N, int Nreal, int R, int S,
                           int stride, int pad_t, int pad_l, int upsample, int splits, int dtype, void* stream);

int ddpm_wgrad_effective_splits(int K, int splits, int dtype);

int ddpm_conv3x3_wgrad_splits(int B, int H, int W, int C, int N, int splits);
int ddpm_conv3x3_wgrad_nhwc(const void* dy, long long dy_ld, const void* x, long long x_ld, float* dw, long long slab_stride,
                            float* dbias, long long bias_stride, int B, int H, int W, int C, int N, int Nreal, int splits,
                            int dtype, void* stream);
int ddpm_conv3x3_wgrad_up_nhwc(const void* dy, long long dy_ld, const void* x, long long x_ld, float* dw, long long slab_stride,
                               float* dbias, long long bias_stride, int B, int H, int W, int C, int N, int Nreal, int splits,
                               int dtype, void* stream);

int ddpm_conv1x1_wgrad_splits(int P, int C, int N);
int ddpm_conv1x1_wgrad_nhwc(const void* dy, long long dy_ld, const void* x, long long x_ld, float* dw, long long slab_stride,
                            float* dbias, long long bias_stride, int P, int C, int N, int splits, int dtype, void* stream);

int ddpm_wgrad_reduce(const long long* table, int n_tensors, void* stream);

int ddpm_wgrad_unpack(const float* gpack, float* gflat, const long long* descs, int n_tensors, float scale, void* stream);
int ddpm_wgrad_unpack_sumsq(const float* gpack, float* gflat, const long long* descs, int n_tensors, float scale, float* total_sq,
                            long long total_sq_floats, void* stream);

int ddpm_gemm(const void* a, long long a_ld, long long a_bs, int a_trans,
              const void* b, long long b_ld, long long b_bs, int b_trans,
              void* c, long long c_ld, long long c_bs,
              const float* bias, const void* residual, long long res_ld, long long res_bs,
              int M, int N, int K, int batch, float alpha, int accumulate, int out_mode, int splits,
              int dtype, void* stream);

int ddpm_attention_fwd(const void* qkv, long long ld, void* out, long long out_ld, int B, int L, int C, float scale,
                       int dtype, void* stream);

int ddpm_attention_fwd_lse(const void* qkv, long long ld, void* out, long long out_ld, float* lse, int B, int L, int C, float scale,
                           int dtype, void* stream);
int ddpm_attention_bwd(const void* qkv, long long ld, const void* o, long long o_ld, const void* d_o, long long do_ld,
                       const float* lse, float* dvec, void* dqkv, long long dqkv_ld, int B, int L, int C, float scale,
                       int dtype, void* stream);

int ddpm_groupnorm_silu_fwd(const void* x, long long x_ld, void* y, long long y_ld, const float* gamma, const float* beta,
                            float* stats, float* workspace, int B, int HW, int C, int G, float eps, int silu,
                            float drop_p, unsigned long long seed, const unsigned long long* seed_dev, int dtype, void* stream);
int ddpm_groupnorm_silu_bwd(const void* x, long long x_ld, const void* dy, long long dy_ld, void* dx, long long dx_ld,
                            const float* gamma, const float* beta, const float* stats, float* dgamma, float* dbeta,
                            float* workspace, int B, int HW, int C, int G, int silu, float drop_p, unsigned long long seed,
                            const unsigned long long* seed_dev, int accumulate, float* dx_colsum, long long colsum_ld,
                            const void* add, long long add_ld, int dtype, void* stream);
long long ddpm_gn_workspace_floats(int B, int HW, int C, int G, int dtype);

int ddpm_timestep_embedding(const long long* t, const float* freqs, float* out, int B, int dim, void* stream);

int ddpm_nchw_to_nhwc(const float* x, void* y, int B, int C, int HW, int Cp, int dtype, void* stream);
int ddpm_pack_weight(const float* w, void* w_fwd , void* w_dgrad ,
                     int N, int C, int R, int S, int Cp, int Np, int dtype, void* stream);

int ddpm_pack_weight_multi(const long long* descs, int n_tensors, int dtype, void* stream);

int ddpm_q_sample(const float* x0, const float* noise, const long long* t, const float* sqrt_ab, const float* sqrt_1mab,
                  float* xt, int B, int n, int T, void* stream);
int ddpm_mse_fwd(const float* pred, const float* target, float* loss, int B, int n, void* stream);
int ddpm_mse_bwd(const float* pred, const float* target, const float* gloss, float* gpred, int B, int n, void* stream);
int ddpm_weighted_sum_f32(const float* x, const float* w, float* out, int n, void* stream);
int ddpm_atb_f32(const float* a, long long lda, const float* b, long long ldb, float* c, long long ldc, int M, int N, int K, void* stream);
int ddpm_p_sample_step(const float* x_t, const float* model_out, const float* z, const long long* t,
                       const float* sqrt_recip_ab, const float* sqrt_recip_m1_ab, const float* post_coef1, const float* post_coef2,
                       const float* logvar, float* x_prev, float* pred_x0, int B, int n, int mean_type, int clip, int T, void* stream);
int ddpm_vlb_terms(const float* x_0, const float* x_t, const float* model_out, const long long* t,
                   const float* sqrt_recip_ab, const float* sqrt_recip_m1_ab, const float* post_coef1, const float* post_coef2,
                   const float* post_logvar, const float* model_logvar, float* loss, float* pred_x0,
                   int B, int n, int mean_type, int clip, int T, void* stream);
int ddpm_vlb_terms_bwd(const float* x_0, const float* x_t, const float* model_out, const long long* t,
                       const float* sqrt_recip_ab, const float* sqrt_recip_m1_ab, const float* post_coef1, const float* post_coef2,
                       const float* post_logvar, const float* model_logvar, const float* gloss, float* gout,
                       int B, int n, int mean_type, int T, void* stream);
int ddpm_gather_i64(const long long* idx, const long long* map, long long* out, int B, void* stream);
int ddpm_add_i64(long long* t, int B, long long delta, void* stream);
int ddpm_gather_rows_f32(const float* table, const long long* idx, float* out, int rows, int row_len, int table_rows, void* stream);

int ddpm_silu_fwd(const float* x, float* y, long long n, void* stream);
int ddpm_silu_bwd(const float* x, const float* dy, float* dx, long long n, int accumulate, void* stream);

int ddpm_colsum(const void* dy, long long ld, float* per_sample, long long ps_ld, float* total, int B, int HW, int C, int dtype, void* stream);
int ddpm_upsample2x_bwd(const void* dy_up, void* dx, long long dx_ld, int B, int H, int W, int C, int accumulate, int dtype, void* stream);
int ddpm_resample2x_nhwc(const void* x, long long x_ld, void* y, long long y_ld, int B, int H, int W, int C, int up, float scale,
                         int accumulate, int dtype, void* stream);
int ddpm_add_rows(const void* x, long long x_ld, void* y, long long y_ld, long long rows, int C, int accumulate, int dtype, void* stream);

int ddpm_softmax_fwd(const float* s, void* p, long long rows, int L, int dtype, void* stream);
int ddpm_softmax_bwd(const void* p, const float* dp, void* ds, long long rows, int L, int dtype, void* stream);

int ddpm_sumsq_accumulate(const float* g, long long n, float* total_sq, float* workspace, void* stream);
int ddpm_adam_ema_step(float* p, const float* g, float* m, float* v, float* shadow, long long n, const float* total_sq,
                       float max_norm, float lr, float beta1, float beta2, float eps, float bias_corr1, float bias_corr2,
                       float ema_w, void* stream);

int ddpm_mt_sumsq_slots(int n_tensors);
int ddpm_mt_grad_sumsq(const long long* table, int n_tensors, float* total_sq, long long total_sq_floats, void* stream);
int ddpm_mt_adam_ema(const long long* table, int n_tensors, const float* total_sq, float max_norm, float lr, float beta1,
                     float beta2, float eps, float bias_corr1, float bias_corr2, float ema_w, const float* hyper_dev, void* stream);

int ddpm_mt_gather_f32(const long long* table, int n_tensors, void* stream);

int ddpm_toy_time_table(const float* freqs, const float* tproj_w, const float* tproj_b, const float* enc_w, const float* enc_b,
                        float* tabs, int T, int M, void* stream);
int ddpm_toy_decoder_fwd(const float* x, const long long* t, const float* w_in, const float* n1_w, const float* n1_b, const float* fc1_w,
                         const float* n2_w, const float* n2_b, const float* fc2_w, const float* on_w, const float* on_b, const float* out_w,
                         const float* out_b, const float* tabs, float* y, float* saved, int B, int D, int M, int L, int T, void* stream);
int ddpm_toy_decoder_bwd(const float* x, const long long* t, const float* dy, const float* w_in, const float* n1_w, const float* n1_b,
                         const float* fc1_w, const float* n2_w, const float* n2_b, const float* fc2_w, const float* on_w, const float* on_b,
                         const float* out_w, const float* tabs, const float* saved, float* dx, float* grads, float* dzsum, float* ws,
                         long long ws_floats, int B, int D, int M, int L, int T, void* stream);
int ddpm_toy_time_table_bwd(const long long* t, const float* dzsum, const float* freqs, const float* enc_w, const float* tabs, float* gtab,
                            float* ws, long long ws_floats, int B, int M, int T, void* stream);

int ddpm_manifold_kth_f16(const void* rows, long long rows_ld, int Nr, const void* cols, long long cols_ld, int Nc, int D, int rank,
                          void* out, void* workspace, long long workspace_bytes, void* stream);
int ddpm_manifold_cover_f16(const void* probe, long long probe_ld, int Np, const void* support, long long support_ld, int Ns, int D,
                            const void* support_kth, void* hit, void* workspace, long long workspace_bytes, void* stream);

int ddpm_stream_order(void* waiter, void* signaller);
int ddpm_fill_zero(void* p, long long bytes, void* stream);
void* ddpm_plan_create(void);
int ddpm_plan_destroy(void* plan);
int ddpm_plan_append(void* plan, const char* entry, const unsigned long long* words, int n_words);
int ddpm_plan_cut(void* plan);
int ddpm_plan_segments(void* plan);
int ddpm_plan_entries(void* plan);
int ddpm_plan_run(void* plan, int segment);
const char* ddpm_plan_failed_entry(void* plan, int* index);
int ddpm_plan_entry_arity(const char* entry);

#ifdef __cplusplus
}
#endif
#endif
```

include/ddpm_hip_debug.h:

```cpp
#ifndef DDPM_HIP_DEBUG_H
#define DDPM_HIP_DEBUG_H
#ifdef __cplusplus
extern "C" {
#endif

int ddpm_conv2d_variant(long long x_ld, long long y_ld, int B, int H, int W, int C, int Ho, int Wo, int N, int R, int S,
                        int stride, int pad_t, int pad_l, int upsample, int dilate, int out_mode, int splits, int dtype, int epilogue);
int ddpm_conv2d_wgrad_variant(long long dy_ld, long long x_ld, int B, int H, int W, int C, int Creal, int Ho, int Wo, int N, int Nreal,
                              int R, int S, int stride, int pad_t, int pad_l, int upsample, int splits, int dtype);
int ddpm_gemm_variant(long long a_ld, int a_trans, long long b_ld, int b_trans, long long c_ld, int M, int N, int K, int batch,
                      int out_mode, int splits, int dtype);
int ddpm_conv3x3_wgrad_variant(int B, int H, int W, int C, int N);

int ddpm_mfma_probe(float* sink, int iters, int zero_operands, void* stream);

int ddpm_conv3x3_pc_last_fault(unsigned* out4);
int ddpm_wgrad3x3_ws_last_fault(unsigned* out4);

int ddpm_set_reserved_cus(int n);
int ddpm_get_reserved_cus(void);
int ddpm_copy_probe(void* dst, const void* src, long long bytes, int blocks, void* stream);

int ddpm_dropout_mask(float* mask, long long n, float p, unsigned long long seed, void* stream);

#ifdef __cplusplus
}
#endif
#endif
```

Before: 14570 imgs/s.

## Fuse gradient unpack, Adam+EMA update and weight repack into one plan kernel

```diff
diff --git a/ddpm-torch_amd/csrc/common.h b/ddpm-torch_amd/csrc/common.h
--- a/ddpm-torch_amd/csrc/common.h
+++ b/ddpm-torch_amd/csrc/common.h
@@ -119,6 +119,25 @@
     return s * (1.0f + z * (1.0f - s));
 }
 
+struct AdamEmaCoef {
+    float clip, beta1, beta2, step, sqrt_bc2, eps, ema_w;
+};
+__device__ __forceinline__ void adam_ema_update(float& pi, float gi, float& mi, float& vi, float& si, const AdamEmaCoef& k) {
+    gi *= k.clip;
+    mi = k.beta1 * mi + (1.f - k.beta1) * gi;
+    vi = k.beta2 * vi + (1.f - k.beta2) * gi * gi;
+    const float denom = sqrtf(vi) / k.sqrt_bc2 + k.eps;
+    pi = pi - k.step * (mi / denom);
+    si += k.ema_w * (pi - si);
+}
+__device__ __forceinline__ float clip_from_bank(const float* __restrict__ total_sq, float max_norm) {
+    if (!total_sq || !(max_norm > 0.f)) return 1.f;
+    float tot = 0.f;
+    for (int i = 0; i < 64; ++i) tot += total_sq[i];
+    const float c = max_norm / (sqrtf(tot) + 1e-6f);
+    return c < 1.f ? c : 1.f;
+}
+
 #include <atomic>
 struct DevOnce {
     std::atomic<unsigned long long> mask{0};
@@ -153,6 +172,9 @@
 static inline bool aligned16(const void* p) { return (((uintptr_t)p) & 15) == 0; }
 
 int ddpm_sumsq_finish_launch(const float* partial, int n, float* total_sq, void* stream);
+int ddpm_fused_update_launch(const float* gpack, const long long* descs, int n_unpack, float scale, float* total_sq, const long long* rows,
+                             const void* items, int n_items, float max_norm, float lr, float beta1, float beta2, float eps, float bias_corr1,
+                             float bias_corr2, float ema_w, const float* hyper_dev, int dtype, void* stream);
 int ddpm_reserved_cus();
 static inline int ddpm_cu_budget(int wanted) { const int left = 256 - ddpm_reserved_cus(); return wanted < left ? wanted : (left > 1 ? left : 1); }
 int ddpm_pointwise_launch(const void* x, long long x_ld, const void* w, void* y, long long y_ld, const float* bias, const void* residual,
diff --git a/ddpm-torch_amd/csrc/elementwise.hip b/ddpm-torch_amd/csrc/elementwise.hip
--- a/ddpm-torch_amd/csrc/elementwise.hip
+++ b/ddpm-torch_amd/csrc/elementwise.hip
@@ -84,6 +84,75 @@
 template <> __device__ __forceinline__ void pk_store2<bf16_t>(bf16_t* p, float a, float b) { *reinterpret_cast<unsigned*>(p) = pack_bf2(a, b); }
 template <> __device__ __forceinline__ void pk_store2<float>(float* p, float a, float b) { *reinterpret_cast<float2*>(p) = make_float2(a, b); }
 
+template <typename T, int RS>
+__device__ __forceinline__ void pack_tile_store(const float* tile, T* __restrict__ wf, T* __restrict__ wd, int N, int C, int Cp, int Np, bool up_dgrad,
+                                                int n0, int c0) {
+    constexpr int pitch = PK_T * RS + 1;
+    const int tid = threadIdx.x;
+    constexpr bool BF = sizeof(T) == 2;
+    if (wf) {
+        if constexpr (BF) {
+            for (int i = tid; i < PK_T * RS * (PK_T / 8); i += 256) {
+                const int cl = (i % (PK_T / 8)) * 8, r1 = i / (PK_T / 8), tap = r1 % RS, nl = r1 / RS;
+                if (n0 + nl < N && c0 + cl < Cp) {
+                    const float* t8 = tile + nl * pitch + cl * RS + tap;
+                    u32x4 o;
+                    o.x = pack_bf2(t8[0], t8[RS]); o.y = pack_bf2(t8[2 * RS], t8[3 * RS]); o.z = pack_bf2(t8[4 * RS], t8[5 * RS]); o.w = pack_bf2(t8[6 * RS], t8[7 * RS]);
+                    *reinterpret_cast<u32x4*>(wf + ((long long)(n0 + nl) * RS + tap) * Cp + c0 + cl) = o;
+                }
+            }
+        } else {
+            for (int i = tid; i < PK_T * RS * (PK_T / 2); i += 256) {
+                const int cl = (i % (PK_T / 2)) * 2, r1 = i / (PK_T / 2), tap = r1 % RS, nl = r1 / RS;
+                if (n0 + nl < N && c0 + cl < Cp)
+                    pk_store2<T>(wf + ((long long)(n0 + nl) * RS + tap) * Cp + c0 + cl, tile[nl * pitch + cl * RS + tap], tile[nl * pitch + (cl + 1) * RS + tap]);
+            }
+        }
+    }
+    if constexpr (RS == 9) {
+        if (wd && up_dgrad) {
+            for (int i = tid; i < PK_T * 16 * (PK_T / 2); i += 256) {
+                const int nl = (i % (PK_T / 2)) * 2, r1 = i / (PK_T / 2), tap = r1 % 16, cl = r1 / 16;
+                if (c0 + cl >= C || n0 + nl >= Np) continue;
+                const int P = tap >> 2, Q = tap & 3;
+                float acc0 = 0.f, acc1 = 0.f;
+#pragma unroll
+                for (int a = 0; a < 2; ++a)
+#pragma unroll
+                    for (int b2 = 0; b2 < 2; ++b2) {
+                        const int r = P - a, s2 = Q - b2;
+                        if (r >= 0 && r < 3 && s2 >= 0 && s2 < 3) {
+                            acc0 += tile[nl * pitch + cl * 9 + (8 - (r * 3 + s2))];
+                            acc1 += tile[(nl + 1) * pitch + cl * 9 + (8 - (r * 3 + s2))];
+                        }
+                    }
+                pk_store2<T>(wd + ((long long)(c0 + cl) * 16 + tap) * Np + n0 + nl, acc0, acc1);
+            }
+            return;
+        }
+    }
+    if (wd) {
+        if constexpr (BF) {
+            for (int i = tid; i < PK_T * RS * (PK_T / 8); i += 256) {
+                const int nl = (i % (PK_T / 8)) * 8, r1 = i / (PK_T / 8), tap = r1 % RS, cl = r1 / RS;
+                if (c0 + cl < C && n0 + nl < Np) {
+                    const float* t8 = tile + nl * pitch + cl * RS + (RS - 1 - tap);
+                    u32x4 o;
+                    o.x = pack_bf2(t8[0], t8[pitch]); o.y = pack_bf2(t8[2 * pitch], t8[3 * pitch]); o.z = pack_bf2(t8[4 * pitch], t8[5 * pitch]);
+                    o.w = pack_bf2(t8[6 * pitch], t8[7 * pitch]);
+                    *reinterpret_cast<u32x4*>(wd + ((long long)(c0 + cl) * RS + tap) * Np + n0 + nl) = o;
+                }
+            }
+        } else {
+            for (int i = tid; i < PK_T * RS * (PK_T / 2); i += 256) {
+                const int nl = (i % (PK_T / 2)) * 2, r1 = i / (PK_T / 2), tap = r1 % RS, cl = r1 / RS;
+                if (c0 + cl < C && n0 + nl < Np)
+                    pk_store2<T>(wd + ((long long)(c0 + cl) * RS + tap) * Np + n0 + nl, tile[nl * pitch + cl * RS + (RS - 1 - tap)],
+                                 tile[(nl + 1) * pitch + cl * RS + (RS - 1 - tap)]);
+            }
+        }
+    }
+}
 template <typename T, int RS>
 __device__ __forceinline__ void pack_tensor(const float* __restrict__ w, T* __restrict__ wf, T* __restrict__ wd, int N, int C, int Cp, int Np, bool up_dgrad,
                                             float* tile) {
@@ -118,69 +187,7 @@
             }
         }
         __syncthreads();
-        constexpr bool BF = sizeof(T) == 2;
-        if (wf) {
-            if constexpr (BF) {
-                for (int i = tid; i < PK_T * RS * (PK_T / 8); i += 256) {
-                    const int cl = (i % (PK_T / 8)) * 8, r1 = i / (PK_T / 8), tap = r1 % RS, nl = r1 / RS;
-                    if (n0 + nl < N && c0 + cl < Cp) {
-                        const float* t8 = tile + nl * pitch + cl * RS + tap;
-                        u32x4 o;
-                        o.x = pack_bf2(t8[0], t8[RS]); o.y = pack_bf2(t8[2 * RS], t8[3 * RS]); o.z = pack_bf2(t8[4 * RS], t8[5 * RS]); o.w = pack_bf2(t8[6 * RS], t8[7 * RS]);
-                        *reinterpret_cast<u32x4*>(wf + ((long long)(n0 + nl) * RS + tap) * Cp + c0 + cl) = o;
-                    }
-                }
-            } else {
-                for (int i = tid; i < PK_T * RS * (PK_T / 2); i += 256) {
-                    const int cl = (i % (PK_T / 2)) * 2, r1 = i / (PK_T / 2), tap = r1 % RS, nl = r1 / RS;
-                    if (n0 + nl < N && c0 + cl < Cp)
-                        pk_store2<T>(wf + ((long long)(n0 + nl) * RS + tap) * Cp + c0 + cl, tile[nl * pitch + cl * RS + tap], tile[nl * pitch + (cl + 1) * RS + tap]);
-                }
-            }
-        }
-        if constexpr (RS == 9) {
-            if (wd && up_dgrad) {
-                for (int i = tid; i < PK_T * 16 * (PK_T / 2); i += 256) {
-                    const int nl = (i % (PK_T / 2)) * 2, r1 = i / (PK_T / 2), tap = r1 % 16, cl = r1 / 16;
-                    if (c0 + cl >= C || n0 + nl >= Np) continue;
-                    const int P = tap >> 2, Q = tap & 3;
-                    float acc0 = 0.f, acc1 = 0.f;
-#pragma unroll
-                    for (int a = 0; a < 2; ++a)
-#pragma unroll
-                        for (int b2 = 0; b2 < 2; ++b2) {
-                            const int r = P - a, s2 = Q - b2;
-                            if (r >= 0 && r < 3 && s2 >= 0 && s2 < 3) {
-                                acc0 += tile[nl * pitch + cl * 9 + (8 - (r * 3 + s2))];
-                                acc1 += tile[(nl + 1) * pitch + cl * 9 + (8 - (r * 3 + s2))];
-                            }
-                        }
-                    pk_store2<T>(wd + ((long long)(c0 + cl) * 16 + tap) * Np + n0 + nl, acc0, acc1);
-                }
-                continue;
-            }
-        }
-        if (wd) {
-            if constexpr (BF) {
-                for (int i = tid; i < PK_T * RS * (PK_T / 8); i += 256) {
-                    const int nl = (i % (PK_T / 8)) * 8, r1 = i / (PK_T / 8), tap = r1 % RS, cl = r1 / RS;
-                    if (c0 + cl < C && n0 + nl < Np) {
-                        const float* t8 = tile + nl * pitch + cl * RS + (RS - 1 - tap);
-                        u32x4 o;
-                        o.x = pack_bf2(t8[0], t8[pitch]); o.y = pack_bf2(t8[2 * pitch], t8[3 * pitch]); o.z = pack_bf2(t8[4 * pitch], t8[5 * pitch]);
-                        o.w = pack_bf2(t8[6 * pitch], t8[7 * pitch]);
-                        *reinterpret_cast<u32x4*>(wd + ((long long)(c0 + cl) * RS + tap) * Np + n0 + nl) = o;
-                    }
-                }
-            } else {
-                for (int i = tid; i < PK_T * RS * (PK_T / 2); i += 256) {
-                    const int nl = (i % (PK_T / 2)) * 2, r1 = i / (PK_T / 2), tap = r1 % RS, cl = r1 / RS;
-                    if (c0 + cl < C && n0 + nl < Np)
-                        pk_store2<T>(wd + ((long long)(c0 + cl) * RS + tap) * Np + n0 + nl, tile[nl * pitch + cl * RS + (RS - 1 - tap)],
-                                     tile[(nl + 1) * pitch + cl * RS + (RS - 1 - tap)]);
-                }
-            }
-        }
+        pack_tile_store<T, RS>(tile, wf, wd, N, C, Cp, Np, up_dgrad, n0, c0);
     }
 }
 template <typename T>
@@ -207,6 +214,7 @@
     return check_launch();
 }
 
+template <bool STORE>
 __global__ __launch_bounds__(256) void wgrad_unpack_kernel(const float* __restrict__ gpack, float* __restrict__ gflat, const long long* __restrict__ descs, float scale,
                                                             float* __restrict__ sumsq) {
     __shared__ float sh[4];
@@ -219,7 +227,8 @@
     if (RS == 1) {
         for (unsigned i = blockIdx.x * blockDim.x + threadIdx.x; i < total; i += gridDim.x * blockDim.x) {
             const float v = src[i] * scale;
-            dst[i] = v; acc += v * v;
+            if (STORE) dst[i] = v;
+            acc += v * v;
         }
     } else if (RS == 9 && C % 64 == 0) {
         __shared__ float slab[4][64 * 9];
@@ -231,19 +240,25 @@
 #pragma unroll
             for (int tap = 0; tap < 9; ++tap) v[tap] = src[((unsigned long long)n * 9 + tap) * C + c0 + lane] * scale;
 #pragma unroll
-            for (int tap = 0; tap < 9; ++tap) { mine[lane * 9 + tap] = v[tap]; acc += v[tap] * v[tap]; }
-            __builtin_amdgcn_wave_barrier();
-            float* out = dst + ((unsigned long long)n * C + c0) * 9;
-#pragma unroll
-            for (int k = 0; k < 9; ++k) out[k * 64 + lane] = mine[k * 64 + lane];
-            __builtin_amdgcn_wave_barrier();
+            for (int tap = 0; tap < 9; ++tap) {
+                if (STORE) mine[lane * 9 + tap] = v[tap];
+                acc += v[tap] * v[tap];
+            }
+            if (STORE) {
+                __builtin_amdgcn_wave_barrier();
+                float* out = dst + ((unsigned long long)n * C + c0) * 9;
+#pragma unroll
+                for (int k = 0; k < 9; ++k) out[k * 64 + lane] = mine[k * 64 + lane];
+                __builtin_amdgcn_wave_barrier();
+            }
         }
     } else {
         for (unsigned i = blockIdx.x * blockDim.x + threadIdx.x; i < total; i += gridDim.x * blockDim.x) {
             const unsigned nc = i / RS, tap = i - nc * RS;
             const unsigned n = nc / C, c = nc - n * C;
             const float v = src[((unsigned long long)n * RS + tap) * C + c] * scale;
-            dst[i] = v; acc += v * v;
+            if (STORE) dst[i] = v;
+            acc += v * v;
         }
     }
     if (sumsq) {
@@ -256,7 +271,7 @@
 extern "C" int ddpm_wgrad_unpack(const float* gpack, float* gflat, const long long* descs, int n_tensors, float scale, void* stream) {
     if (!gpack || !gflat || !descs) return DDPM_ERR_NULL;
     if (n_tensors <= 0) return DDPM_OK;
-    hipLaunchKernelGGL(wgrad_unpack_kernel, dim3(64, n_tensors), dim3(256), 0, (hipStream_t)stream, gpack, gflat, descs, scale, (float*)nullptr);
+    hipLaunchKernelGGL(wgrad_unpack_kernel<true>, dim3(64, n_tensors), dim3(256), 0, (hipStream_t)stream, gpack, gflat, descs, scale, (float*)nullptr);
     return check_launch();
 }
 extern "C" int ddpm_wgrad_unpack_sumsq(const float* gpack, float* gflat, const long long* descs, int n_tensors, float scale, float* total_sq,
@@ -264,9 +279,139 @@
     if (!gpack || !gflat || !descs || !total_sq) return DDPM_ERR_NULL;
     if (n_tensors <= 0) return DDPM_OK;
     if (total_sq_floats < 64 + 64ll * n_tensors) return DDPM_ERR_SHAPE;
-    hipLaunchKernelGGL(wgrad_unpack_kernel, dim3(64, n_tensors), dim3(256), 0, (hipStream_t)stream, gpack, gflat, descs, scale, total_sq + 64);
+    hipLaunchKernelGGL(wgrad_unpack_kernel<true>, dim3(64, n_tensors), dim3(256), 0, (hipStream_t)stream, gpack, gflat, descs, scale, total_sq + 64);
     const int rc = check_launch();
     return rc ? rc : ddpm_sumsq_finish_launch(total_sq + 64, 64 * n_tensors, total_sq, stream);
+}
+
+constexpr int FU_ROW = 12, FU_CHUNK = 4096;
+
+template <typename T, int RS>
+__device__ __forceinline__ void fused_update_tile(const long long* __restrict__ row, int t, float scale, const AdamEmaCoef& k, float* tile) {
+    constexpr int pitch = PK_T * RS + 1;
+    float* __restrict__ p = reinterpret_cast<float*>(row[0]);
+    const float* __restrict__ g = reinterpret_cast<const float*>(row[1]);
+    float* __restrict__ m = reinterpret_cast<float*>(row[2]);
+    float* __restrict__ v = reinterpret_cast<float*>(row[3]);
+    float* __restrict__ shadow = reinterpret_cast<float*>(row[4]);
+    T* wf = reinterpret_cast<T*>(row[5]);
+    T* wd = reinterpret_cast<T*>(row[6]);
+    const int N = (int)row[7], C = (int)row[8], Cp = (int)row[9], Np = (int)row[10];
+    const bool up_dgrad = ((int)row[11] & 0x100) != 0;
+    const int tiles_c = (Cp + PK_T - 1) / PK_T;
+    const int n0 = (t / tiles_c) * PK_T, c0 = (t % tiles_c) * PK_T;
+    const int cw = min(PK_T, C - c0);
+    const int tid = threadIdx.x;
+    constexpr int KG = PK_T * PK_T * RS / 256;
+    float gv[KG];
+#pragma unroll
+    for (int j = 0; j < KG; ++j) {
+        const int i = tid + 256 * j, cl = i & (PK_T - 1), r1 = i / PK_T, nl = r1 / RS, tap = r1 - nl * RS;
+        gv[j] = n0 + nl < N && cl < cw ? g[((long long)(n0 + nl) * RS + tap) * C + c0 + cl] * scale : 0.f;
+    }
+#pragma unroll
+    for (int j = 0; j < KG; ++j) {
+        const int i = tid + 256 * j, cl = i & (PK_T - 1), r1 = i / PK_T, nl = r1 / RS, tap = r1 - nl * RS;
+        tile[nl * pitch + cl * RS + tap] = gv[j];
+    }
+    __syncthreads();
+    const unsigned long long al = reinterpret_cast<unsigned long long>(p) | reinterpret_cast<unsigned long long>(m) | reinterpret_cast<unsigned long long>(v) |
+                                  reinterpret_cast<unsigned long long>(shadow);
+    const bool vec_ok = ((long long)C * RS) % 4 == 0 && (al & 15) == 0;
+    constexpr int V = PK_T * RS / 4, KV = PK_T * V / 256;
+    if (cw == PK_T && vec_ok) {
+#pragma unroll 3
+        for (int j = 0; j < KV; ++j) {
+            const int i = tid + 256 * j, nl = i / V, q = i - nl * V;
+            if (n0 + nl >= N) continue;
+            const long long at = ((long long)(n0 + nl) * C + c0) * RS + 4 * q;
+            float4 p4 = *reinterpret_cast<float4*>(p + at), m4 = *reinterpret_cast<float4*>(m + at), v4 = *reinterpret_cast<float4*>(v + at);
+            float4 s4 = shadow ? *reinterpret_cast<float4*>(shadow + at) : make_float4(0.f, 0.f, 0.f, 0.f);
+            float* t4 = tile + nl * pitch + 4 * q;
+            adam_ema_update(p4.x, t4[0], m4.x, v4.x, s4.x, k); adam_ema_update(p4.y, t4[1], m4.y, v4.y, s4.y, k);
+            adam_ema_update(p4.z, t4[2], m4.z, v4.z, s4.z, k); adam_ema_update(p4.w, t4[3], m4.w, v4.w, s4.w, k);
+            *reinterpret_cast<float4*>(p + at) = p4; *reinterpret_cast<float4*>(m + at) = m4; *reinterpret_cast<float4*>(v + at) = v4;
+            if (shadow) *reinterpret_cast<float4*>(shadow + at) = s4;
+            t4[0] = p4.x; t4[1] = p4.y; t4[2] = p4.z; t4[3] = p4.w;
+        }
+    } else if (cw > 0) {
+        for (int i = tid; i < PK_T * PK_T * RS; i += 256) {
+            const int nl = i / (PK_T * RS), rem = i - nl * (PK_T * RS);
+            if (n0 + nl >= N || rem >= cw * RS) continue;
+            const long long at = ((long long)(n0 + nl) * C + c0) * RS + rem;
+            float pi = p[at], mi = m[at], vi = v[at], si = shadow ? shadow[at] : 0.f;
+            adam_ema_update(pi, tile[nl * pitch + rem], mi, vi, si, k);
+            p[at] = pi; m[at] = mi; v[at] = vi;
+            if (shadow) shadow[at] = si;
+            tile[nl * pitch + rem] = pi;
+        }
+    }
+    if (!wf && !wd) return;
+    __syncthreads();
+    pack_tile_store<T, RS>(tile, wf, wd, N, C, Cp, Np, up_dgrad, n0, c0);
+}
+
+__device__ __forceinline__ void fused_update_chunk(const long long* __restrict__ row, int chunk, float scale, const AdamEmaCoef& k) {
+    const long long first = (long long)chunk * FU_CHUNK, left = row[7] - first;
+    const int cnt = (int)(left < FU_CHUNK ? left : FU_CHUNK);
+    float* __restrict__ p = reinterpret_cast<float*>(row[0]) + first;
+    const float* __restrict__ g = reinterpret_cast<const float*>(row[1]) + first;
+    float* __restrict__ m = reinterpret_cast<float*>(row[2]) + first;
+    float* __restrict__ v = reinterpret_cast<float*>(row[3]) + first;
+    float* __restrict__ shadow = row[4] ? reinterpret_cast<float*>(row[4]) + first : nullptr;
+    const unsigned long long al = reinterpret_cast<unsigned long long>(p) | reinterpret_cast<unsigned long long>(g) | reinterpret_cast<unsigned long long>(m) |
+                                  reinterpret_cast<unsigned long long>(v) | reinterpret_cast<unsigned long long>(shadow);
+    const int nv = (al & 15) == 0 ? cnt >> 2 : 0;
+    for (int i = threadIdx.x; i < nv; i += 256) {
+        float4 p4 = reinterpret_cast<float4*>(p)[i], m4 = reinterpret_cast<float4*>(m)[i], v4 = reinterpret_cast<float4*>(v)[i];
+        const float4 g4 = reinterpret_cast<const float4*>(g)[i];
+        float4 s4 = shadow ? reinterpret_cast<float4*>(shadow)[i] : make_float4(0.f, 0.f, 0.f, 0.f);
+        adam_ema_update(p4.x, g4.x * scale, m4.x, v4.x, s4.x, k); adam_ema_update(p4.y, g4.y * scale, m4.y, v4.y, s4.y, k);
+        adam_ema_update(p4.z, g4.z * scale, m4.z, v4.z, s4.z, k); adam_ema_update(p4.w, g4.w * scale, m4.w, v4.w, s4.w, k);
+        reinterpret_cast<float4*>(p)[i] = p4; reinterpret_cast<float4*>(m)[i] = m4; reinterpret_cast<float4*>(v)[i] = v4;
+        if (shadow) reinterpret_cast<float4*>(shadow)[i] = s4;
+    }
+    for (int i = (nv << 2) + threadIdx.x; i < cnt; i += 256) {
+        float pi = p[i], mi = m[i], vi = v[i], si = shadow ? shadow[i] : 0.f;
+        adam_ema_update(pi, g[i] * scale, mi, vi, si, k);
+        p[i] = pi; m[i] = mi; v[i] = vi;
+        if (shadow) shadow[i] = si;
+    }
+}
+
+template <typename T>
+__global__ __launch_bounds__(256) void fused_update_kernel(const long long* __restrict__ rows, const int2* __restrict__ items, float scale,
+                                                            const float* __restrict__ total_sq, float max_norm, float lr, float beta1, float beta2,
+                                                            float eps, float bc1, float bc2, float ema_w, const float* __restrict__ hyper) {
+    if (hyper) { lr = hyper[0]; bc1 = hyper[1]; bc2 = hyper[2]; ema_w = hyper[3]; }
+    __shared__ float tile[PK_T * (PK_T * 9 + 1)];
+    const int2 it = items[blockIdx.x];
+    const long long* row = rows + FU_ROW * (long long)it.x;
+    const AdamEmaCoef k = {clip_from_bank(total_sq, max_norm), beta1, beta2, lr / bc1, sqrtf(bc2), eps, ema_w};
+    const int rs = (int)row[11] & 0xff;
+    if (rs == 9) fused_update_tile<T, 9>(row, it.y, scale, k, tile);
+    else if (rs == 1) fused_update_tile<T, 1>(row, it.y, scale, k, tile);
+    else if (rs == 4) fused_update_tile<T, 4>(row, it.y, scale, k, tile);
+    else fused_update_chunk(row, it.y, scale, k);
+}
+int ddpm_fused_update_launch(const float* gpack, const long long* descs, int n_unpack, float scale, float* total_sq, const long long* rows,
+                             const void* items, int n_items, float max_norm, float lr, float beta1, float beta2, float eps, float bias_corr1,
+                             float bias_corr2, float ema_w, const float* hyper_dev, int dtype, void* stream) {
+    if (!gpack || !descs || !total_sq || !rows || !items) return DDPM_ERR_NULL;
+    if (n_unpack <= 0 || n_items <= 0) return DDPM_ERR_SHAPE;
+    if (dtype != DDPM_BF16 && dtype != DDPM_F32) return DDPM_ERR_DTYPE;
+    hipLaunchKernelGGL(wgrad_unpack_kernel<false>, dim3(64, n_unpack), dim3(256), 0, (hipStream_t)stream, gpack, (float*)nullptr, descs, scale, total_sq + 64);
+    int rc = check_launch();
+    if (rc) return rc;
+    rc = ddpm_sumsq_finish_launch(total_sq + 64, 64 * n_unpack, total_sq, stream);
+    if (rc) return rc;
+    if (dtype == DDPM_BF16)
+        hipLaunchKernelGGL(fused_update_kernel<bf16_t>, dim3(n_items), dim3(256), 0, (hipStream_t)stream, rows, (const int2*)items, scale, (const float*)total_sq,
+                           max_norm, lr, beta1, beta2, eps, bias_corr1, bias_corr2, ema_w, hyper_dev);
+    else
+        hipLaunchKernelGGL(fused_update_kernel<float>, dim3(n_items), dim3(256), 0, (hipStream_t)stream, rows, (const int2*)items, scale, (const float*)total_sq,
+                           max_norm, lr, beta1, beta2, eps, bias_corr1, bias_corr2, ema_w, hyper_dev);
+    return check_launch();
 }
 
 __global__ __launch_bounds__(256) void wgrad_reduce_kernel(const long long* __restrict__ table) {
diff --git a/ddpm-torch_amd/csrc/optim.hip b/ddpm-torch_amd/csrc/optim.hip
--- a/ddpm-torch_amd/csrc/optim.hip
+++ b/ddpm-torch_amd/csrc/optim.hip
@@ -36,17 +36,13 @@
         const float c = max_norm / (sqrtf(total_sq[0]) + 1e-6f);
         clip = c < 1.f ? c : 1.f;
     }
-    const float step = lr / bc1;
-    const float sqrt_bc2 = sqrtf(bc2);
+    const AdamEmaCoef k = {clip, beta1, beta2, lr / bc1, sqrtf(bc2), eps, ema_w};
     for (long long i = (long long)blockIdx.x * blockDim.x + threadIdx.x; i < n; i += (long long)gridDim.x * blockDim.x) {
-        const float gi = g[i] * clip;
-        const float mi = beta1 * m[i] + (1.f - beta1) * gi;
-        const float vi = beta2 * v[i] + (1.f - beta2) * gi * gi;
+        float pi = p[i], mi = m[i], vi = v[i], si = shadow ? shadow[i] : 0.f;
+        adam_ema_update(pi, g[i], mi, vi, si, k);
         m[i] = mi; v[i] = vi;
-        const float denom = sqrtf(vi) / sqrt_bc2 + eps;
-        const float pi = p[i] - step * (mi / denom);
         p[i] = pi;
-        if (shadow) shadow[i] += ema_w * (pi - shadow[i]);
+        if (shadow) shadow[i] = si;
     }
 }
 extern "C" int ddpm_adam_ema_step(float* p, const float* g, float* m, float* v, float* shadow, long long n, const float* total_sq,
@@ -106,23 +102,8 @@
     float* v = reinterpret_cast<float*>(row[3]);
     float* shadow = reinterpret_cast<float*>(row[4]);
     const long long n = row[5];
-    float clip = 1.f;
-    if (total_sq && max_norm > 0.f) {
-        float tot = 0.f;
-        for (int i = 0; i < MT_SUMSQ_LANES; ++i) tot += total_sq[i];
-        const float c = max_norm / (sqrtf(tot) + 1e-6f);
-        clip = c < 1.f ? c : 1.f;
-    }
-    const float step = lr / bc1;
-    const float sqrt_bc2 = sqrtf(bc2);
-    auto upd = [&](float& pi, float gi, float& mi, float& vi, float& si) {
-        gi *= clip;
-        mi = beta1 * mi + (1.f - beta1) * gi;
-        vi = beta2 * vi + (1.f - beta2) * gi * gi;
-        const float denom = sqrtf(vi) / sqrt_bc2 + eps;
-        pi = pi - step * (mi / denom);
-        si += ema_w * (pi - si);
-    };
+    const AdamEmaCoef k = {clip_from_bank(total_sq, max_norm), beta1, beta2, lr / bc1, sqrtf(bc2), eps, ema_w};
+    auto upd = [&](float& pi, float gi, float& mi, float& vi, float& si) { adam_ema_update(pi, gi, mi, vi, si, k); };
     const unsigned long long al = reinterpret_cast<unsigned long long>(p) | reinterpret_cast<unsigned long long>(g) | reinterpret_cast<unsigned long long>(m) |
                                   reinterpret_cast<unsigned long long>(v) | reinterpret_cast<unsigned long long>(shadow);
     const long long nv = (al & 15) == 0 ? n >> 2 : 0;
diff --git a/ddpm-torch_amd/csrc/plan.hip b/ddpm-torch_amd/csrc/plan.hip
--- a/ddpm-torch_amd/csrc/plan.hip
+++ b/ddpm-torch_amd/csrc/plan.hip
@@ -2,6 +2,7 @@
 #include "../../include/ddpm_hip.h"
 #include "../../include/ddpm_hip_debug.h"
 
+#include <algorithm>
 #include <cstring>
 #include <mutex>
 #include <type_traits>
@@ -66,7 +67,15 @@
 };
 constexpr int kNumEntryPoints = (int)(sizeof(kEntryPoints) / sizeof(kEntryPoints[0]));
 
-enum Mode : unsigned char { RUN, PRODUCER, WAIT, RECORD, SKIP };
+enum Mode : unsigned char { RUN, PRODUCER, WAIT, RECORD, SKIP, FUSED };
+
+struct FusedUpdate {
+    int head = -1;
+    void* dev = nullptr;
+    const long long* rows = nullptr;
+    const void* items = nullptr;
+    int n_items = 0;
+};
 
 struct Entry {
     thunk_t thunk;
@@ -81,6 +90,7 @@
     std::vector<word_t> words;
     std::vector<int> segment_end;
     std::vector<hipEvent_t> bound;
+    std::vector<FusedUpdate> fused;
     size_t resolved_entries = 0, resolved_cuts = 0;
     int failed_index = -1;
     int failed_status = 0;
@@ -148,6 +158,164 @@
     p->resolved_cuts = p->segment_end.size();
 }
 
+
+constexpr int kFuRow = 12, kFuChunk = 4096, kFuTile = 32;
+
+int entry_point_index(const char* name) {
+    for (int i = 0; i < kNumEntryPoints; ++i)
+        if (std::strcmp(kEntryPoints[i].name, name) == 0) return i;
+    return -1;
+}
+
+bool fetch_table(std::vector<long long>& host, word_t dev, long long n_rows, int width) {
+    if (!dev || n_rows <= 0 || n_rows > (1 << 20)) return false;
+    host.resize((size_t)n_rows * width);
+    if (hipMemcpy(host.data(), reinterpret_cast<const void*>(static_cast<uintptr_t>(dev)), host.size() * sizeof(long long), hipMemcpyDeviceToHost) != hipSuccess) {
+        (void)hipGetLastError();
+        return false;
+    }
+    return true;
+}
+
+bool fuse(Plan* p, int head, FusedUpdate& out) {
+    const word_t* wu = p->words.data() + p->entries[head].first_word;
+    const word_t* wa = p->words.data() + p->entries[head + 1].first_word;
+    const word_t* wp = p->words.data() + p->entries[head + 2].first_word;
+    const long long nu = from_word<int>(wu[3]), na = from_word<int>(wa[1]), np = from_word<int>(wp[1]);
+    const int dtype = from_word<int>(wp[2]);
+    if (wu[7] != wa[12] || wu[7] != wp[3]) return false;
+    if (!wu[0] || !wu[1] || !wu[5] || wu[5] != wa[2]) return false;
+    if (from_word<long long>(wu[6]) < 64 + 64 * nu) return false;
+    if (dtype != DDPM_BF16 && dtype != DDPM_F32) return false;
+    if (hipDeviceSynchronize() != hipSuccess) { (void)hipGetLastError(); return false; }
+    std::vector<long long> U, A, P;
+    if (!fetch_table(U, wu[2], nu, 5) || !fetch_table(A, wa[0], na, 6) || !fetch_table(P, wp[0], np, 8)) return false;
+    const long long gpack = (long long)wu[0], gflat = (long long)wu[1];
+    const long long lim = (1ll << 31) - 1;
+    for (long long u = 0; u < nu; ++u) {
+        const long long* d = &U[5 * u];
+        if (d[0] < 0 || d[1] < 0 || d[2] <= 0 || d[3] <= 0 || d[4] <= 0 || d[2] * d[3] > lim || d[2] * d[3] * d[4] > lim) return false;
+    }
+    std::vector<char> pack_used((size_t)np, 0);
+    std::vector<long long> rows;
+    std::vector<int> items;
+    std::vector<std::pair<long long, std::pair<int, int>>> order;
+    for (long long a = 0; a < na; ++a) {
+        const long long* r = &A[6 * a];
+        const long long n = r[5];
+        if (n <= 0) continue;
+        if (n > lim || !r[0] || !r[1] || !r[2] || !r[3]) return false;
+        int owner = -1;
+        for (long long u = 0; u < nu; ++u) {
+            const long long* d = &U[5 * u];
+            const long long lo = gflat + 4 * d[1], hi = lo + 4 * d[2] * d[3] * d[4];
+            if (r[1] >= lo && r[1] + 4 * n <= hi) {
+                if (owner >= 0) return false;
+                owner = (int)u;
+            }
+        }
+        if (owner < 0) return false;
+        const long long* d = &U[5 * owner];
+        const long long rs_u = d[4], within = (r[1] - (gflat + 4 * d[1])) / 4;
+        if (rs_u > 1 && (within != 0 || n != d[2] * d[3] * rs_u)) return false;
+        int pk = -1;
+        for (long long q = 0; q < np; ++q)
+            if (P[8 * q] == r[0]) {
+                if (pk >= 0 || pack_used[q]) return false;
+                pk = (int)q;
+            }
+        long long row[kFuRow] = {r[0], gpack + 4 * (d[0] + within), r[2], r[3], r[4], 0, 0, n, 0, 0, 0, 0};
+        long long n_items = 0, cost = 0;
+        if (pk >= 0 || rs_u > 1) {
+            long long N = d[2], C = d[3], Cp = C, Np = N, rs = rs_u, flags = 0;
+            if (pk >= 0) {
+                const long long* q = &P[8 * pk];
+                const long long R = q[5] & 0xff;
+                N = q[3]; C = q[4]; Cp = q[6]; Np = q[7]; rs = R * R; flags = q[5] & 0x100;
+                if (N <= 0 || C <= 0 || N * C * rs != n || Cp < C || Np < N || Cp > lim || Np > lim || (!q[1] && !q[2])) return false;
+                if (rs_u > 1 ? (rs != rs_u || N != d[2] || C != d[3]) : rs != 1) return false;
+                if (flags && rs != 9) return false;
+                row[5] = q[1]; row[6] = q[2];
+                pack_used[pk] = 1;
+            }
+            if (rs != 9 && rs != 4 && rs != 1) return false;
+            row[7] = N; row[8] = C; row[9] = Cp; row[10] = Np; row[11] = rs | flags;
+            n_items = ((Cp + kFuTile - 1) / kFuTile) * ((Np + kFuTile - 1) / kFuTile);
+            cost = kFuTile * kFuTile * rs;
+        } else {
+            n_items = (n + kFuChunk - 1) / kFuChunk;
+            cost = kFuChunk;
+        }
+        if (n_items > lim || (long long)order.size() + n_items > (1 << 24)) return false;
+        const int ri = (int)(rows.size() / kFuRow);
+        rows.insert(rows.end(), row, row + kFuRow);
+        for (long long t = 0; t < n_items; ++t) order.push_back({-cost, {ri, (int)t}});
+    }
+    for (long long q = 0; q < np; ++q)
+        if (!pack_used[q]) return false;
+    if (order.empty()) return false;
+    std::stable_sort(order.begin(), order.end(), [](const auto& x, const auto& y) { return x.first < y.first; });
+    for (const auto& o : order) { items.push_back(o.second.first); items.push_back(o.second.second); }
+    const size_t row_bytes = rows.size() * sizeof(long long), item_bytes = items.size() * sizeof(int);
+    void* dev = nullptr;
+    if (hipMalloc(&dev, row_bytes + item_bytes) != hipSuccess) { (void)hipGetLastError(); return false; }
+    if (hipMemcpy(dev, rows.data(), row_bytes, hipMemcpyHostToDevice) != hipSuccess ||
+        hipMemcpy(static_cast<char*>(dev) + row_bytes, items.data(), item_bytes, hipMemcpyHostToDevice) != hipSuccess) {
+        (void)hipGetLastError();
+        (void)hipFree(dev);
+        return false;
+    }
+    out.head = head;
+    out.dev = dev;
+    out.rows = static_cast<const long long*>(dev);
+    out.items = static_cast<const char*>(dev) + row_bytes;
+    out.n_items = (int)order.size();
+    return true;
+}
+
+void drop_fused(Plan* p) {
+    for (FusedUpdate& f : p->fused)
+        if (f.dev) (void)hipFree(f.dev);
+    p->fused.clear();
+}
+
+void prepare(Plan* p) {
+    drop_fused(p);
+    resolve(p);
+    static const int ep_unpack = entry_point_index("ddpm_wgrad_unpack_sumsq"), ep_adam = entry_point_index("ddpm_mt_adam_ema"),
+                     ep_pack = entry_point_index("ddpm_pack_weight_multi");
+    const int n = (int)p->entries.size();
+    size_t seg = 0;
+    int end = 0;
+    for (int i = 0; i + 2 < n; ++i) {
+        while (end <= i) end = seg < p->segment_end.size() ? p->segment_end[seg++] : n;
+        Entry* e = &p->entries[i];
+        if (i + 2 >= end || e[0].ep != ep_unpack || e[1].ep != ep_adam || e[2].ep != ep_pack) continue;
+        if (e[0].mode != RUN || e[1].mode != RUN || e[2].mode != RUN) continue;
+        FusedUpdate f;
+        if (!fuse(p, i, f)) continue;
+        e[0].mode = FUSED;
+        e[0].producer = (int)p->fused.size();
+        e[1].mode = e[2].mode = SKIP;
+        p->fused.push_back(f);
+        i += 2;
+    }
+}
+
+int run_fused(const Plan* p, const Entry& e) {
+    const FusedUpdate& f = p->fused[e.producer];
+    const word_t* wu = p->words.data() + e.first_word;
+    const word_t* wa = p->words.data() + (&e)[1].first_word;
+    const word_t* wp = p->words.data() + (&e)[2].first_word;
+    return ddpm_fused_update_launch(from_word<const float*>(wu[0]), from_word<const long long*>(wu[2]), from_word<int>(wu[3]), from_word<float>(wu[4]),
+                                    from_word<float*>(wu[5]), f.rows, f.items, f.n_items, from_word<float>(wa[3]), from_word<float>(wa[4]),
+                                    from_word<float>(wa[5]), from_word<float>(wa[6]), from_word<float>(wa[7]), from_word<float>(wa[8]),
+                                    from_word<float>(wa[9]), from_word<float>(wa[10]), from_word<const float*>(wa[11]), from_word<int>(wp[2]),
+                                    from_word<void*>(wu[7]));
+}
+
+inline bool stale(const Plan* p) { return p->resolved_entries != p->entries.size() || p->resolved_cuts != p->segment_end.size(); }
+
 }
 
 thread_local DdpmLaunchEdge g_ddpm_launch_edge;
@@ -171,8 +339,22 @@
 void* ddpm_plan_create(void) { return new Plan(); }
 
 int ddpm_plan_destroy(void* plan) {
+    if (plan) drop_fused(static_cast<Plan*>(plan));
     delete static_cast<Plan*>(plan);
     return DDPM_OK;
+}
+
+int ddpm_plan_prepare(void* plan) {
+    if (!plan) return DDPM_ERR_NULL;
+    Plan* p = static_cast<Plan*>(plan);
+    if (stale(p)) prepare(p);
+    return DDPM_OK;
+}
+
+int ddpm_plan_fused_updates(void* plan) {
+    if (!plan) return -DDPM_ERR_NULL;
+    Plan* p = static_cast<Plan*>(plan);
+    return stale(p) ? 0 : (int)p->fused.size();
 }
 
 int ddpm_plan_append(void* plan, const char* entry, const unsigned long long* words, int n_words) {
@@ -216,7 +398,7 @@
     if (segment < 0 || segment > closed) return DDPM_ERR_SHAPE;
     const int first = segment ? p->segment_end[segment - 1] : 0;
     const int last = segment < closed ? p->segment_end[segment] : (int)p->entries.size();
-    if (p->resolved_entries != p->entries.size() || p->resolved_cuts != p->segment_end.size()) resolve(p);
+    if (stale(p)) prepare(p);
     const word_t* words = p->words.data();
     const Entry* e = p->entries.data();
     EventRing* ring = nullptr;
@@ -228,6 +410,8 @@
             rc = e[i].thunk(w);
         } else if (e[i].mode == SKIP) {
             continue;
+        } else if (e[i].mode == FUSED) {
+            rc = run_fused(p, e[i]);
         } else {
             if (!ring && !(ring = ring_of_device())) rc = DDPM_ERR_LAUNCH;
             else if (e[i].mode == PRODUCER) {
diff --git a/ddpm-torch_amd/ddpm_torch/_hip.py b/ddpm-torch_amd/ddpm_torch/_hip.py
--- a/ddpm-torch_amd/ddpm_torch/_hip.py
+++ b/ddpm-torch_amd/ddpm_torch/_hip.py
@@ -86,7 +86,9 @@
     "ddpm_plan_cut": [P],
     "ddpm_plan_segments": [P],
     "ddpm_plan_entries": [P],
+    "ddpm_plan_prepare": [P],
     "ddpm_plan_run": [P, I],
+    "ddpm_plan_fused_updates": [P],
     "ddpm_plan_failed_entry": [P, P],
     "ddpm_plan_entry_arity": [ctypes.c_char_p],
 }
diff --git a/ddpm-torch_amd/ddpm_torch/_plan.py b/ddpm-torch_amd/ddpm_torch/_plan.py
--- a/ddpm-torch_amd/ddpm_torch/_plan.py
+++ b/ddpm-torch_amd/ddpm_torch/_plan.py
@@ -92,6 +92,13 @@
                     raise RuntimeError(f"ddpm_plan_append({name}) failed: the executor does not know this entry point with {len(w)} arguments")
             if i + 1 < len(self.segments):
                 lib.ddpm_plan_cut(self._c)
+        rc = lib.ddpm_plan_prepare(self._c)
+        if rc != 0:
+            raise RuntimeError(f"ddpm_plan_prepare failed: {_hip._ERR.get(rc, rc)}")
+
+    @property
+    def fused_updates(self):
+        return 0 if self._c is None else int(_hip.lib().ddpm_plan_fused_updates(self._c))
 
     def replay(self):
         if self._c is not None:
diff --git a/include/ddpm_hip.h b/include/ddpm_hip.h
--- a/include/ddpm_hip.h
+++ b/include/ddpm_hip.h
@@ -140,6 +140,7 @@
 int ddpm_plan_cut(void* plan);
 int ddpm_plan_segments(void* plan);
 int ddpm_plan_entries(void* plan);
+int ddpm_plan_prepare(void* plan);
 int ddpm_plan_run(void* plan, int segment);
 const char* ddpm_plan_failed_entry(void* plan, int* index);
 int ddpm_plan_entry_arity(const char* entry);
diff --git a/include/ddpm_hip_debug.h b/include/ddpm_hip_debug.h
--- a/include/ddpm_hip_debug.h
+++ b/include/ddpm_hip_debug.h
@@ -23,6 +23,8 @@
 
 int ddpm_dropout_mask(float* mask, long long n, float p, unsigned long long seed, void* stream);
 
+int ddpm_plan_fused_updates(void* plan);
+
 #ifdef __cplusplus
 }
 #endif
```

New measurement: 14710 imgs/s (median of 6 runs). No clear change (+0.9%).
